# huyhoang17/DB_text_minimal

Measured on AMD Instinct MI355X. Metric: train images/sec @640x640 bs=16/GPU, higher is better.
Workload: dtype f32

## Files before the change

db_text_minimal_amd/_lib.py:

```python
import ctypes
import os
import subprocess

_HERE = os.path.dirname(os.path.abspath(__file__))
LIB_PATH = os.environ.get('DBN_LIB_PATH') or os.path.join(_HERE, 'libdbnet_hip.so')
CSRC = os.path.join(_HERE, 'csrc')

_P, _I, _L, _F = ctypes.c_void_p, ctypes.c_int, ctypes.c_long, ctypes.c_float

SIGNATURES = {
    'dbn_pack_weights': 'piiiiiipp',
    'dbn_igemm_panel_floats': 'iiiiii',
    'dbn_igemm_packed_floats': 'ii',
    'dbn_igemm_f32': 'pppp' + 'i' * 14 + 'p',
    'dbn_igemm_tile_config': 'ii',
    'dbn_igemm_tile_config_ns': 'iii',
    'dbn_conv_bn_ws_floats': 'iiiiii',
    'dbn_pack_weights_batched': 'piip',
    'dbn_igemm_splitk_plan': 'iiii',
    'dbn_igemm_splitk_plan_ns': 'iiiii',
    'dbn_igemm_splitk_f32': 'pppp' + 'i' * 16 + 'pp',
    'dbn_deform_im2col': 'ppp' + 'i' * 11 + 'p',
    'dbn_deform_col2im': 'ppppp' + 'i' + 'p' + 'i' * 11 + 'p',
    'dbn_deform_col2im_ws_bytes': 'i' * 8,
# ... 46 lines not shown
    'dbn_detect_poly': 'piiiifi' + 'pppppp',
    'dbn_detect_poly_host': 'ppppp' + 'iiii' + 'pp' + 'pppi' + 'pppp',
    'dbn_det_eval_ws_bytes': 'i',
    'dbn_det_eval_overlaps': 'ppipilippppp',
    'dbn_det_eval_match_host': 'ii' + 'p' * 12,
    'dbn_pyramid_conv_ws_floats': 'iiii',
    'dbn_pyramid_conv_f32': 'p' * 10 + 'i' * 7 + 'pp' + 'ff' + 'ppppppp' + 'p',
    'dbn_conv_bn_f32': 'pppp' + 'i' * 15 + 'pp' + 'ff' + 'ppppppp' + 'p',
    'dbn_pack_weights_bf16s': 'piiiiiiipp',
    'dbn_igemm_bf16s_panel_floats': 'iiiiiii',
    'dbn_igemm_bf16s': 'pppp' + 'i' * 15 + 'p',
    'dbn_wgrad_bf16s': 'pppp' + 'i' * 12 + 'fip',
    'dbn_wgrad_splitk': 'iiiiiii',
    'dbn_wgrad_slab_floats': 'iiiiiii',
    'dbn_wgrad_splitk_hw': 'iiiiiiiii',
    'dbn_wgrad_slab_floats_hw': 'iiiiiiiiii',
    'dbn_set_index_limits': 'lll',
    'dbn_wgrad_f32': 'pppp' + 'i' * 12 + 'fp',
    'dbn_reduce_ws_floats': 'i',
    'dbn_bn_train_stats': 'piippffppppppp' + 'p',
    'dbn_bn_eval_coef': 'ippppfppp',
    'dbn_bn_apply': 'pppppppliip',
    'dbn_bn_backward': 'pppppppp' + 'pp' + 'i' + 'pp' + 'ii' + 'f' + 'pp',
    'dbn_bn_backward_from_sums': 'ppppppppp' + 'pp' + 'i' + 'pp' + 'ii' + 'f' + 'pp',
    'dbn_bn_backward_ex': 'ppppppppp' + 'pp' + 'i' + 'ppp' + 'ii' + 'f' + 'pp',
    'dbn_col_sum': 'piipfpp',
    'dbn_bnrelu_maxpool_fwd': 'ppppiiiip',
    'dbn_bnrelu_maxpool_bwd': 'ppppppiiiip',
    'dbn_nearest_up_fwd': 'ppp' + 'i' * 8 + 'p',
    'dbn_nearest_up_bwd': 'pp' + 'i' * 9 + 'p',
    'dbn_bilinear_fwd': 'ppliiiip',
    'dbn_bilinear_bwd': 'ppliiiip',
    'dbn_fpn_combine_weights': 'piiiipp',
    'dbn_fpn_scatter_wgrad': 'ppppiipp',
    'dbn_nchw3_to_nhwc4': 'ppiiip',
    'dbn_add_inplace': 'pplp',
    'dbn_head_tail_fwd': 'p' * 11 + 'iiii' + 'f' + 'p',
    'dbn_head_tail_bwd_ws_floats': '',
    'dbn_head_tail_bwd': 'p' * 21 + 'iiii' + 'ff' + 'pp',
    'dbn_db_loss_ws_bytes': '',
    'dbn_db_loss_fwd': 'pp' + 'iiii' + 'ffff' + 'pppp',
    'dbn_db_loss_sum_fwd': 'pp' + 'iiii' + 'ffff' + 'pppp',
    'dbn_db_loss_frac_fwd': 'pp' + 'iiii' + 'ffff' + 'i' + 'pppp',
    'dbn_db_loss_bwd': 'pppp' + 'ff' + 'iiii' + 'pp',
    'dbn_db_loss_ohem_ws_bytes': 'iii',
    'dbn_db_loss_ohem_fwd': 'pp' + 'iiii' + 'ffff' + 'pppp',
    'dbn_db_loss_ohem_bwd': 'ppppp' + 'ff' + 'iiii' + 'pp',
    'dbn_pixel_confusion': 'plppiiifpp',
    'dbn_adam_step': 'pppp' + 'l' + 'ffff' + 'i' + 'f' + 'p',
    'dbn_clock_probe': 'pip',
    'dbn_has_experiments': '',
    'dbn_wall_clock_khz': '',
}
SIGNATURES.update({
    'dbn_igemm_t': 'ii' + 'pppp' + 'i' * 14 + 'i' + 'p' + 'p',
    'dbn_conv_bn_t': 'i' + SIGNATURES['dbn_conv_bn_f32'],
    'dbn_pyramid_conv_t': 'i' + SIGNATURES['dbn_pyramid_conv_f32'],
    'dbn_pyramid_conv_from_t': 'ii' + SIGNATURES['dbn_pyramid_conv_f32'],
    'dbn_igemm_bn_rows': 'i' * 15,
    'dbn_igemm_bnsums_t': 'ii' + 'pppp' + 'i' * 14 + 'ppppppp' + 'pppp' + 'p' + 'p',
    'dbn_igemm_bn_final_counters': 'ii',
    'dbn_igemm_bn_final_group_floats': 'ii',
    'dbn_wgrad_t': 'ii' + 'pppp' + 'i' * 12 + 'f' + 'p',
    'dbn_wgrad_phase_t': 'iii' + 'pppp' + 'i' * 12 + 'f' + 'p',
    'dbn_wgrad_reduce_describe': 'ii' + 'pppp' + 'i' * 12 + 'f' + 'p',
    'dbn_wgrad_reduce_many': 'ppiiip',
    'dbn_wgrad_tile_config': 'ii',
    'dbn_set_wgrad_variant': 'i',
    'dbn_set_convt_kernel': 'i',
    'dbn_igemm_splitk_slab_floats': 'iiiii',
    'dbn_wgrad_kernel_config': 'iiiii',
    'dbn_wgrad_kernel_config_hw': 'i' * 12,
    'dbn_set_patch_conv': 'i',
    'dbn_set_wres16': 'i',
    'dbn_set_pyramid_wide': 'i',
    'dbn_pyramid_wide_would_run': 'iiiiii',
    'dbn_conv_bn_set_final': 'pp',
    'dbn_conv_bn_final_group_doubles': 'ii',
    'dbn_wres16_would_run': 'iiiiiiiii',
    'dbn_mfma_sustained': 'ippip',
    'dbn_mfma_sustained_flops': 'ii',
    'dbn_set_stagger': 'i',
    'dbn_winograd_eligible': 'iiiii',
    'dbn_winograd_panel_floats': 'ii',
    'dbn_winograd_pack': 'piiiipp',
    'dbn_winograd_rows': 'iii',
    'dbn_winograd_pack_batched': 'pip',
    'dbn_winograd_dgrad_bnsums_f32': 'ppp' + 'iiiiii' + 'pppp' + 'ppp' + 'pppp' + 'p' + 'p',
    'dbn_winograd_ws_floats': 'iiii',
    'dbn_winograd_wgrad_eligible': 'iiiiii',
    'dbn_winograd_wgrad_linear': 'ii',
    'dbn_winograd_wgrad_slab_floats': 'iiiii',
    'dbn_winograd_wgrad_f32': 'ipppppp' + 'iiiiii' + 'fp',
    'dbn_winograd_conv_bn_act_f32': 'pppppp' + 'iiiii' + 'pp' + 'ff' + 'ppppppp' + 'p',
    'dbn_winograd_conv_bn_f32': 'pppp' + 'iiiii' + 'pp' + 'ff' + 'ppppppp' + 'p',
    'dbn_set_phase_priority': 'i',
    'dbn_set_winograd_persistent': 'i',
    'dbn_set_winograd_stagger': 'i',
    'dbn_set_winograd_blocks_per_barrier': 'i',
    'dbn_fold_bn_eval': 'pilppppp' + 'f' + 'ppp',
    'dbn_igemm_act_t': 'ii' + 'pppp' + 'i' + 'p' + 'i' * 13 + 'p',
    'dbn_winograd_conv_act_f32': 'pppp' + 'i' + 'p' + 'iiiii' + 'p',
    'dbn_pyramid_conv_act_t': 'ii' + 'p' * 9 + 'i' + 'p' + 'i' * 6 + 'p',
    'dbn_set_trace': 'pl',
    'dbn_igemm_kernel_config': 'i' * 16,
    'dbn_split3': 'pplp',
    'dbn_deform_im2col_t': 'i' + SIGNATURES['dbn_deform_im2col'],
    'dbn_deform_col2im_t': 'i' + SIGNATURES['dbn_deform_col2im'],
    'dbn_deform_col2im_gather_t': 'i' + SIGNATURES['dbn_deform_col2im'],
    'dbn_deform_col2im_gather_ws_bytes': 'iii',
    'dbn_deform_offset_absmax_t': 'iplpp',
    'dbn_pw16_eligible': 'iiiiii',
    'dbn_pw16_panel_bytes': '',
    'dbn_pw16_pack': 'ipipp',
    'dbn_pw16_act_t': 'ipppipiiiip',
    'dbn_set_head_tail_wide': 'i',
    'dbn_stem16_pool_eligible': 'iiii',
    'dbn_stem16_conv_bn_relu_pool_t': 'ipppppiiip',
    'dbn_head16_eligible': 'iiii',
    'dbn_head16_tail_eval_t': 'i' + 'p' * 15 + 'iii' + 'p',
    'dbn_cast_f32': 'ipplp',
    'dbn_pack_weights_t': 'ip' + 'i' * 7 + 'pp',
    'dbn_igemm_panel_floats_t': 'i' * 8,
    'dbn_bn_train_stats_t': 'i' + SIGNATURES['dbn_bn_train_stats'],
    'dbn_bn_apply_t': 'i' + SIGNATURES['dbn_bn_apply'],
    'dbn_bn_backward_t': 'ipi' + SIGNATURES['dbn_bn_backward_ex'][1:],
    'dbn_col_sum_t': 'i' + SIGNATURES['dbn_col_sum'],
    'dbn_bnrelu_maxpool_fwd_t': 'i' + SIGNATURES['dbn_bnrelu_maxpool_fwd'],
    'dbn_bnrelu_maxpool_bwd_t': 'i' + SIGNATURES['dbn_bnrelu_maxpool_bwd'][:-1] + 'pppp',
    'dbn_maxpool_bwd_parts': 'iiii',
    'dbn_bnrelu_maxpool_fwd_arg_t': 'ipppppp' + 'iiii' + 'p',
    'dbn_maxpool_bn_backward_ws_floats': 'iiii',
    'dbn_maxpool_bn_backward_t': 'i' + 'p' * 10 + 'iiii' + 'f' + 'pp',
    'dbn_nearest_up_fwd_t': 'i' + SIGNATURES['dbn_nearest_up_fwd'],
    'dbn_nearest_up_bwd_t': 'i' + SIGNATURES['dbn_nearest_up_bwd'],
    'dbn_nchw3_to_nhwc4_t': 'i' + SIGNATURES['dbn_nchw3_to_nhwc4'],
    'dbn_nchw3_to_nhwc4_packed_t': 'i' + SIGNATURES['dbn_nchw3_to_nhwc4'],
    'dbn_nchw3_to_nhwc16_and_4_t': 'ipppiiip',
    'dbn_convt16_rows': '',
    'dbn_convt16_panel_bytes': '',
    'dbn_convt16_eligible': 'iiiiii',
    'dbn_convt16_pack': 'ippp',
    'dbn_convt16_bn_t': 'ippppiii' + 'pp' + 'ff' + 'ppppppp' + 'p',
    'dbn_stem16_padded_h': 'i',
    'dbn_stem16_padded_w': 'i',
    'dbn_stem16_rows': '',
    'dbn_stem16_panel_bytes': '',
    'dbn_stem16_eligible': 'iiii',
    'dbn_stem16_pack': 'ippp',
    'dbn_nchw3_to_padded4_t': 'ipppiiip',
    'dbn_stem16_conv_bn_t': 'ipppiii' + 'pp' + 'ff' + 'ppppppp' + 'p',
    'dbn_head_tail_fwd_t': 'i' + SIGNATURES['dbn_head_tail_fwd'],
    'dbn_head_tail_bwd_t': 'i' + SIGNATURES['dbn_head_tail_bwd'],
})
LONG_RETURN = {'dbn_jpeg_coef_elems', 'dbn_jpeg_coef_elems_ex', 'dbn_jpeg_dhuff_ws_bytes', 'dbn_jpeg_encode_bound', 'dbn_greedy_decode_ws_bytes', 'dbn_det_eval_ws_bytes', 'dbn_detect_ws_bytes', 'dbn_detect_poly_ws_bytes', 'dbn_detect_poly_verts_cap', 'dbn_mfma_sustained_flops', 'dbn_conv_bn_final_group_doubles', 'dbn_maxpool_bn_backward_ws_floats', 'dbn_pw16_panel_bytes', 'dbn_stem16_panel_bytes', 'dbn_convt16_panel_bytes', 'dbn_winograd_panel_floats', 'dbn_winograd_wgrad_slab_floats', 'dbn_winograd_ws_floats', 'dbn_igemm_splitk_slab_floats', 'dbn_deform_col2im_ws_bytes', 'dbn_deform_col2im_gather_ws_bytes', 'dbn_igemm_bn_final_counters', 'dbn_igemm_bn_final_group_floats', 'dbn_igemm_panel_floats_t', 'dbn_wgrad_slab_floats_hw', 'dbn_wgrad_slab_floats', 'dbn_igemm_panel_floats', 'dbn_igemm_bf16s_panel_floats', 'dbn_db_loss_ohem_ws_bytes', 'dbn_conv_bn_ws_floats', 'dbn_pyramid_conv_ws_floats'}
_KIND = {'p': _P, 'i': _I, 'l': _L, 'f': _F}


class HipLibraryError(RuntimeError):
    pass


class WgradReduceJob(ctypes.Structure):
    _fields_ = ([('slab', _P), ('grad', _P)] + [(f, _I) for f in ('splitk', 'O', 'J', 'Jp', 'BM', 'BN', 'Cb', 'I', 'RS', 'G', 'natural', 'blocks')]
                + [('scale', _F), ('smem_bytes', _I)])


class BnbFinal(ctypes.Structure):
    _fields_ = [('counters', _P), ('group', _P), ('c1c2', _P), ('dgamma', _P), ('dbeta', _P), ('c1c2_2', _P), ('dgamma_2', _P),
                ('dbeta_2', _P), ('grad_scale', _F)]


def build(verbose=False):
    res = subprocess.run(['make', '-C', CSRC, '-j8'], capture_output=True, text=True)
    if verbose or res.returncode != 0:
        print(res.stdout[-4000:])
        print(res.stderr[-4000:])
    if res.returncode != 0:
        raise HipLibraryError('building libdbnet_hip.so failed (see output above)')
    return LIB_PATH


def source_stamp():
    import hashlib
    h = hashlib.sha256()
    for name in sorted(os.listdir(CSRC)):
        if name.endswith(('.hip', '.h')) or name == 'Makefile':
            h.update(name.encode())
            with open(os.path.join(CSRC, name), 'rb') as f:
                h.update(f.read())
    return h.hexdigest()[:16]


_lib = None


def lib():
    global _lib
    if _lib is None:
        if not os.path.exists(LIB_PATH):
            raise HipLibraryError('%s not found: run `python -c "import __graft_entry__ as g; g.build()"` '
                                  '(there is no CPU fallback for the DBNet hot path)' % LIB_PATH)
        try:
            l = ctypes.CDLL(LIB_PATH)
        except OSError as e:
            raise HipLibraryError('cannot load %s: %s' % (LIB_PATH, e))
        for name, sig in SIGNATURES.items():
            fn = getattr(l, name)
            fn.argtypes = [_KIND[k] for k in sig]
            fn.restype = _L if name in LONG_RETURN else _I
        _lib = l
    return _lib


def check(rc, what=''):
    if rc != 0:
        if rc == 1:
            raise RuntimeError('libdbnet_hip: invalid argument in %s' % what)
        raise RuntimeError('libdbnet_hip: %s failed with hipError %d' % (what, rc - 1000))
```

db_text_minimal_amd/csrc/head_loss.hip:

```cpp
#include "common.h"

namespace {

__device__ __forceinline__ float sigmoidf_(float x) { return 1.f / (1.f + __expf(-x)); }
__device__ __forceinline__ float sigmoid_acc(float x) { return 1.f / (1.f + expf(-x)); }
__device__ __forceinline__ float sigmoid_fast(float x) { return __builtin_amdgcn_rcpf(1.f + __expf(-x)); }

template <int CTRL>
__device__ __forceinline__ float dpp_f32(float v) {
    return __builtin_bit_cast(float, __builtin_amdgcn_update_dpp(0, __builtin_bit_cast(int, v), CTRL, 0xF, 0xF, true));
}
constexpr int DPP_QUAD_XOR1 = 0xB1;
constexpr int DPP_QUAD_XOR2 = 0x4E;
constexpr int DPP_ROW_HALF_MIRROR = 0x141;
constexpr int DPP_ROW_MIRROR = 0x140;
__device__ __forceinline__ float group16_sum(float v) {
    v += dpp_f32<DPP_QUAD_XOR1>(v);
    v += dpp_f32<DPP_QUAD_XOR2>(v);
    v += dpp_f32<DPP_ROW_HALF_MIRROR>(v);
    v += dpp_f32<DPP_ROW_MIRROR>(v);
    return v;
}
#ifndef DBN_HT_NODPP
#define DBN_HT_NODPP 0
#endif
#ifndef DBN_HT_CHECK
#define DBN_HT_CHECK 0
#endif
#ifndef DBN_HT_WAVES
#define DBN_HT_WAVES 0
#endif
template <int K>
__device__ __forceinline__ float quad_bcast(float v) {
#if DBN_HT_NODPP
    return __shfl(v, (int)((threadIdx.x & 63u & ~3u) | K), 64);
#else
    return dpp_f32<K | (K << 2) | (K << 4) | (K << 6)>(v);
#endif
}

__device__ __forceinline__ float group8_sum(float v) {
    v += dpp_f32<DPP_QUAD_XOR1>(v);
    v += dpp_f32<DPP_QUAD_XOR2>(v);
    v += dpp_f32<DPP_ROW_HALF_MIRROR>(v);
    return v;
}

template <int AT, int LPP>
__global__ __launch_bounds__(256) void head_tail_fwd_kernel(const void* __restrict__ xb, const void* __restrict__ xt, const float* __restrict__ wb,
                                     const float* __restrict__ wt, const float* __restrict__ bias_b,
                                     const float* __restrict__ bias_t, const float* __restrict__ sc_b,
                                     const float* __restrict__ sh_b, const float* __restrict__ sc_t,
                                     const float* __restrict__ sh_t, float* __restrict__ out, int N, int Hq, int Wq, int CH,
                                     float kstep, long per) {
    static_assert((LPP == 16) || (LPP == 8 && AT != 0), "eight lanes per pixel: 16-bit storage");
    constexpr int NQ = 16 / LPP;
    const int q = threadIdx.x & (LPP - 1);
    const bool bn = sc_b != nullptr;
    f32x4 scb[NQ], shb[NQ], sct[NQ], sht[NQ];
#pragma unroll
    for (int h = 0; h < NQ; ++h) {
        scb[h] = sct[h] = f32x4{1.f, 1.f, 1.f, 1.f};
        shb[h] = sht[h] = f32x4{0.f, 0.f, 0.f, 0.f};
        if (bn) {
            scb[h] = *reinterpret_cast<const f32x4*>(sc_b + 4 * (NQ * q + h));
            shb[h] = *reinterpret_cast<const f32x4*>(sh_b + 4 * (NQ * q + h));
            sct[h] = *reinterpret_cast<const f32x4*>(sc_t + 4 * (NQ * q + h));
            sht[h] = *reinterpret_cast<const f32x4*>(sh_t + 4 * (NQ * q + h));
        }
    }
    const long npx = (long)N * Hq * Wq;
    const long gstride = blockDim.x / LPP;
    const long r1 = min(npx, (blockIdx.x + 1) * per);
    f32x4 wbq[4 * NQ], wtq[4 * NQ];
#pragma unroll
    for (int e = 0; e < 4 * NQ; ++e) {
        wbq[e] = *reinterpret_cast<const f32x4*>(wb + (4 * NQ * q + e) * 4);
        wtq[e] = *reinterpret_cast<const f32x4*>(wt + (4 * NQ * q + e) * 4);
    }
    const float bb = bias_b[0], bt = bias_t[0];
    const int H = 2 * Hq, W = 2 * Wq;
    const long HW = (long)H * W;
    const long px0 = blockIdx.x * per + (threadIdx.x / LPP);
    const long HWq = (long)Hq * Wq;
    long n = px0 / HWq;
    int hq = (int)((px0 - n * HWq) / Wq), wq = (int)((px0 - n * HWq) - (long)hq * Wq);
    const long g_n = gstride / HWq;
    const int g_h = (int)((gstride - g_n * HWq) / Wq), g_w = (int)((gstride - g_n * HWq) - (long)g_h * Wq);
    auto advance = [&]() {
        wq += g_w;
        if (wq >= Wq) { wq -= Wq; ++hq; }
        hq += g_h;
        if (hq >= Hq) { hq -= Hq; ++n; }
        n += g_n;
    };
    auto load = [&](const void* x, long px, f32x4 (&v)[NQ]) {
        if constexpr (NQ == 1) v[0] = dbn_ld4<AT>(x, px * 16 + q);
        else dbn_ldq<AT>(x, px * 8 + q, v);
    };
    auto finish = [&](f32x4 (&vb)[NQ], f32x4 (&vt)[NQ], long pn, int ph, int pw) {
        if (bn) {
#pragma unroll
            for (int h = 0; h < NQ; ++h)
#pragma unroll
                for (int e = 0; e < 4; ++e) {
                    vb[h][e] = dbn_affine_relu(vb[h][e], scb[h][e], shb[h][e]);
                    vt[h][e] = dbn_affine_relu(vt[h][e], sct[h][e], sht[h][e]);
                }
        }
        f32x4 sb = {0.f, 0.f, 0.f, 0.f}, stt = {0.f, 0.f, 0.f, 0.f};
#pragma unroll
        for (int h = 0; h < NQ; ++h)
#pragma unroll
            for (int e = 0; e < 4; ++e) {
                sb += vb[h][e] * wbq[4 * h + e];
                stt += vt[h][e] * wtq[4 * h + e];
            }
#pragma unroll
        for (int ab = 0; ab < 4; ++ab) {
            sb[ab] = LPP == 16 ? group16_sum(sb[ab]) : group8_sum(sb[ab]);
            stt[ab] = LPP == 16 ? group16_sum(stt[ab]) : group8_sum(stt[ab]);
        }
        if (q < 4) {
            const int ab = q;
            const float lp = (ab == 0 ? sb[0] : ab == 1 ? sb[1] : ab == 2 ? sb[2] : sb[3]) + bb;
            const float lt = (ab == 0 ? stt[0] : ab == 1 ? stt[1] : ab == 2 ? stt[2] : stt[3]) + bt;
            const float P = sigmoid_fast(lp), T = sigmoid_fast(lt);
            const long o = (long)(2 * ph + (ab >> 1)) * W + 2 * pw + (ab & 1);
            float* base = out + pn * CH * HW + o;
            base[0] = P;
            base[HW] = T;
            if (CH == 3) base[2 * HW] = sigmoid_fast(kstep * (P - T));
        }
    };
    long px = px0;
    for (; px + 3 * gstride < r1; px += 4 * gstride) {
        f32x4 vb[4][NQ], vt[4][NQ];
#pragma unroll
        for (int u = 0; u < 4; ++u) {
            load(xb, px + u * gstride, vb[u]);
            load(xt, px + u * gstride, vt[u]);
        }
#pragma unroll
        for (int u = 0; u < 4; ++u) {
            finish(vb[u], vt[u], n, hq, wq);
            advance();
        }
    }
    for (; px < r1; px += gstride, advance()) {
        f32x4 vb[NQ], vt[NQ];
        load(xb, px, vb);
        load(xt, px, vt);
        finish(vb, vt, n, hq, wq);
    }
}

#if DBN_HT_WAVES
#define DBN_HT_OCC __attribute__((amdgpu_waves_per_eu(DBN_HT_WAVES, DBN_HT_WAVES)))
#else
#define DBN_HT_OCC
#endif
template <int AT>
__global__ __launch_bounds__(256) DBN_HT_OCC void head_tail_bwd_kernel(const void* __restrict__ xb, const void* __restrict__ xt, const float* __restrict__ wb,
                                     const float* __restrict__ wt, const float* __restrict__ preds,
                                     const float* __restrict__ dpreds, const float* __restrict__ sc_b,
                                     const float* __restrict__ sh_b, const float* __restrict__ sc_t,
                                     const float* __restrict__ sh_t, const float* __restrict__ mean_b,
                                     const float* __restrict__ rstd_b, const float* __restrict__ mean_t,
                                     const float* __restrict__ rstd_t, void* __restrict__ dxb, void* __restrict__ dxt,
                                     float* __restrict__ part, int N, int Hq, int Wq, int CH, float kstep) {
    const int q = threadIdx.x & 15;
    const int grp = threadIdx.x >> 4;
    const bool bn = sc_b != nullptr;
    f32x4 scb = {1.f, 1.f, 1.f, 1.f}, shb = {0.f, 0.f, 0.f, 0.f}, sct = scb, sht = shb;
    if (bn) {
        scb = *reinterpret_cast<const f32x4*>(sc_b + 4 * q);
        shb = *reinterpret_cast<const f32x4*>(sh_b + 4 * q);
        sct = *reinterpret_cast<const f32x4*>(sc_t + 4 * q);
        sht = *reinterpret_cast<const f32x4*>(sh_t + 4 * q);
    }
    const long npx = (long)N * Hq * Wq;
    const long gstride = (long)gridDim.x * (blockDim.x >> 4);
    f32x4 wbq[4], wtq[4];
#pragma unroll
    for (int e = 0; e < 4; ++e) {
        wbq[e] = *reinterpret_cast<const f32x4*>(wb + (4 * q + e) * 4);
        wtq[e] = *reinterpret_cast<const f32x4*>(wt + (4 * q + e) * 4);
    }
    const bool bnsum = bn && mean_b != nullptr;
    f32x4 mub = {0.f, 0.f, 0.f, 0.f}, rsb = mub, mut = mub, rst = mub;
    if (bnsum) {
        mub = *reinterpret_cast<const f32x4*>(mean_b + 4 * q);
        rsb = *reinterpret_cast<const f32x4*>(rstd_b + 4 * q);
        mut = *reinterpret_cast<const f32x4*>(mean_t + 4 * q);
        rst = *reinterpret_cast<const f32x4*>(rstd_t + 4 * q);
    }
    f32x4 s1b = {0.f, 0.f, 0.f, 0.f}, s2b = s1b, s1t = s1b, s2t = s1b;
    const int H = 2 * Hq, W = 2 * Wq;
    const long HW = (long)H * W;
    f32x4 awb[4], awt[4];
#pragma unroll
    for (int e = 0; e < 4; ++e) {
        awb[e] = f32x4{0.f, 0.f, 0.f, 0.f};
        awt[e] = f32x4{0.f, 0.f, 0.f, 0.f};
    }
    float abb = 0.f, abt = 0.f;
    const long px0 = blockIdx.x * (long)(blockDim.x >> 4) + grp;
    const long HWq = (long)Hq * Wq;
    long n = px0 / HWq;
    int hq = (int)((px0 - n * HWq) / Wq), wq = (int)((px0 - n * HWq) - (long)hq * Wq);
    const long g_n = gstride / HWq;
    const int g_h = (int)((gstride - g_n * HWq) / Wq), g_w = (int)((gstride - g_n * HWq) - (long)g_h * Wq);
    auto advance = [&]() {
        wq += g_w;
        if (wq >= Wq) { wq -= Wq; ++hq; }
        hq += g_h;
        if (hq >= Hq) { hq -= Hq; ++n; }
        n += g_n;
    };
    for (long px = px0; px < npx; px += gstride, advance()) {
        float dlb = 0.f, dlt = 0.f;
        {
            const int ab = q & 3;
            const long o = (long)(2 * hq + (ab >> 1)) * W + 2 * wq + (ab & 1);
            const float* pb = preds + n * CH * HW + o;
            const float* db = dpreds + n * CH * HW + o;
            const float P = pb[0], T = pb[HW];
            float dP = db[0], dT = db[HW];
            if (CH == 3) {
                const float B = pb[2 * HW];
                const float gB = db[2 * HW] * kstep * B * (1.f - B);
                dP += gB;
                dT -= gB;
            }
            dlb = dP * P * (1.f - P);
            dlt = dT * T * (1.f - T);
        }
        const f32x4 lb = {quad_bcast<0>(dlb), quad_bcast<1>(dlb), quad_bcast<2>(dlb), quad_bcast<3>(dlb)};
        const f32x4 lt = {quad_bcast<0>(dlt), quad_bcast<1>(dlt), quad_bcast<2>(dlt), quad_bcast<3>(dlt)};
        f32x4 vb = dbn_ld4<AT>(xb, px * 16 + q);
        f32x4 vt = dbn_ld4<AT>(xt, px * 16 + q);
        const f32x4 yb = vb, yt = vt;
        if (bn) {
#pragma unroll
            for (int e = 0; e < 4; ++e) {
                vb[e] = dbn_affine_relu(vb[e], scb[e], shb[e]);
                vt[e] = dbn_affine_relu(vt[e], sct[e], sht[e]);
            }
        }
        f32x4 gb, gt;
#pragma unroll
        for (int e = 0; e < 4; ++e) {
            gb[e] = wbq[e][0] * lb[0] + wbq[e][1] * lb[1] + wbq[e][2] * lb[2] + wbq[e][3] * lb[3];
            gt[e] = wtq[e][0] * lt[0] + wtq[e][1] * lt[1] + wtq[e][2] * lt[2] + wtq[e][3] * lt[3];
            awb[e] += vb[e] * lb;
            awt[e] += vt[e] * lt;
        }
        dbn_st4<AT>(dxb, px * 16 + q, gb);
        dbn_st4<AT>(dxt, px * 16 + q, gt);
        if (bnsum) {
            if constexpr (AT != 0) {
#pragma unroll
                for (int e = 0; e < 4; ++e) {
                    gb[e] = AT == 1 ? (float)(__bf16)gb[e] : (float)(_Float16)gb[e];
                    gt[e] = AT == 1 ? (float)(__bf16)gt[e] : (float)(_Float16)gt[e];
                }
            }
#pragma unroll
            for (int e = 0; e < 4; ++e) {
                const float mb = vb[e] > 0.f ? gb[e] : 0.f, mt = vt[e] > 0.f ? gt[e] : 0.f;
                s1b[e] += mb;
                s2b[e] += mb * ((yb[e] - mub[e]) * rsb[e]);
                s1t[e] += mt;
                s2t[e] += mt * ((yt[e] - mut[e]) * rst[e]);
            }
        }
        if (q == 0) {
            abb += lb[0] + lb[1] + lb[2] + lb[3];
            abt += lt[0] + lt[1] + lt[2] + lt[3];
        }
    }
#if DBN_HT_CHECK
    {
        float* dbg = part + (long)(2 * 257 + 4 * 64) * gridDim.x;
        int bad_w = 0, bad_t = 0, low_only = 0;
#pragma unroll
        for (int e = 0; e < 4; ++e) {
            const f32x4 a = *reinterpret_cast<const volatile f32x4*>(wb + (4 * q + e) * 4), b = *reinterpret_cast<const volatile f32x4*>(wt + (4 * q + e) * 4);
#pragma unroll
            for (int k = 0; k < 4; ++k) {
                const unsigned ua = __builtin_bit_cast(unsigned, a[k]), ur = __builtin_bit_cast(unsigned, wbq[e][k]);
                bad_w += ua != ur;
                low_only += (ua != ur) && ((ua >> 16) == (ur >> 16));
                bad_t += __builtin_bit_cast(unsigned, b[k]) != __builtin_bit_cast(unsigned, wtq[e][k]);
            }
        }
        int bad_s = 0;
        if (bn) {
            const f32x4 a = *reinterpret_cast<const volatile f32x4*>(sc_b + 4 * q), b = *reinterpret_cast<const volatile f32x4*>(sh_b + 4 * q);
#pragma unroll
            for (int k = 0; k < 4; ++k) bad_s += (__builtin_bit_cast(unsigned, a[k]) != __builtin_bit_cast(unsigned, scb[k])) + (__builtin_bit_cast(unsigned, b[k]) != __builtin_bit_cast(unsigned, shb[k]));
        }
        if (bad_w) atomicAdd(dbg + 0, 1.f);
        if (bad_t) atomicAdd(dbg + 1, 1.f);
        if (bad_s) atomicAdd(dbg + 2, 1.f);
        if (low_only) atomicAdd(dbg + 4, 1.f);
    }
#endif
    constexpr int ROWS = 2 * 257 + 4 * 64;
    __shared__ float red[16][ROWS];
    {
        float* r = red[grp];
#pragma unroll
        for (int e = 0; e < 4; ++e)
#pragma unroll
            for (int ab = 0; ab < 4; ++ab) {
                r[(4 * q + e) * 4 + ab] = awb[e][ab];
                r[257 + (4 * q + e) * 4 + ab] = awt[e][ab];
            }
        if (q == 0) {
            r[256] = abb;
            r[257 + 256] = abt;
        }
#pragma unroll
        for (int e = 0; e < 4; ++e) {
            r[514 + 4 * q + e] = s1b[e];
            r[514 + 64 + 4 * q + e] = s2b[e];
            r[514 + 128 + 4 * q + e] = s1t[e];
            r[514 + 192 + 4 * q + e] = s2t[e];
        }
    }
    __syncthreads();
    for (int i = threadIdx.x; i < ROWS; i += blockDim.x) {
        float s = 0.f;
        for (int g = 0; g < 16; ++g) s += red[g][i];
        part[(long)i * gridDim.x + blockIdx.x] = s;
    }
}

__global__ void fold_partials_d_kernel(const float* __restrict__ part, int nb, int n, float* __restrict__ out, float scale) {
    const int i = blockIdx.x * 8 + (threadIdx.x >> 5);
    const int l32 = threadIdx.x & 31;
    if (i >= n) return;
    const double s = dbn_team32_fold(part, nb, i, l32);
    if (l32 == 0) out[i] = (float)(s * scale);
}

__global__ void fold_head_grads_kernel(const float* __restrict__ part, int nb, float* __restrict__ dw_b, float* __restrict__ dbias_b,
                                       float* __restrict__ dw_t, float* __restrict__ dbias_t, float scale) {
    const int i = blockIdx.x * 8 + (threadIdx.x >> 5);
    const int l32 = threadIdx.x & 31;
    if (i >= 2 * 257) return;
    const double s = dbn_team32_fold(part, nb, i, l32);
    if (l32 != 0) return;
    const int j = i < 257 ? i : i - 257;
    float* dst = i < 257 ? (j < 256 ? dw_b + j : dbias_b) : (j < 256 ? dw_t + j : dbias_t);
    *dst = (float)(s * scale);
}

enum { S_POS = 0, S_NEG, S_BCE, S_L1, S_A, S_BGM, S_BM, S_NONBIN , NSUM };

template <int V>
__device__ __forceinline__ f32x4 ldv(const float* p) {
    if constexpr (V == 4) return *reinterpret_cast<const f32x4*>(p);
    return f32x4{p[0], 0.f, 0.f, 0.f};
}
template <int V>
__device__ __forceinline__ void stv(float* p, f32x4 v) {
    if constexpr (V == 4) *reinterpret_cast<f32x4*>(p) = v;
    else p[0] = v[0];
}



struct DbLossFinal {
    long px;
    int CH;
    float alpha, beta, negative_ratio, eps;
    int bce_sum;
    float* losses;
    float* coef;
    unsigned* counter;
};

__device__ __forceinline__ void db_loss_finish(const double (&s)[NSUM], const DbLossFinal& f) {
    const long n_pos = (long)(float)s[S_POS];
    const long n_neg_expect = (long)((double)n_pos * (double)f.negative_ratio);
    const long n_neg_cur = (long)(float)s[S_NEG];
    const long n_neg = n_neg_expect < n_neg_cur ? n_neg_expect : n_neg_cur;
    const double bce_div = f.bce_sum ? 1.0 : (double)f.px;
    const float bce = (float)(s[S_BCE] / bce_div);
    const float denom = (float)((double)(n_pos + n_neg) + (double)f.eps);
    const float num_w = (float)s[S_POS] + (float)n_neg;
    const float prob = bce * num_w / denom;
    const float thr = (float)s[S_L1] / ((float)s[S_A] + f.eps);
    const float pt = prob + f.beta * thr;
    float* losses = f.losses;
    float* coef = f.coef;
    losses[0] = prob;
    losses[1] = thr;
    coef[0] = num_w / denom / (float)bce_div;
    coef[1] = 1.f / ((float)s[S_A] + f.eps);
    coef[7] = (float)s[S_NONBIN];
    if (f.CH == 3) {
        const float U = (float)s[S_BM] + (float)s[S_POS] + f.eps;
        const float I = (float)s[S_BGM];
        const float binl = 1.f - 2.f * I / U;
        losses[2] = binl;
        losses[3] = pt;
        losses[4] = f.alpha * binl + pt;
        coef[2] = U;
        coef[3] = I;
    } else {
        losses[2] = 0.f;
        losses[3] = pt;
        losses[4] = pt;
        coef[2] = 1.f;
        coef[3] = 0.f;
    }
}

__device__ __forceinline__ void db_loss_fold_and_finish(const double* __restrict__ part, int nb, const DbLossFinal& f, double* red ) {
    constexpr int PER = 4;
    double v[PER][NSUM];
#pragma unroll
    for (int i = 0; i < PER; ++i) {
        const int b = threadIdx.x + i * 256;
#pragma unroll
        for (int k = 0; k < NSUM; ++k)
            v[i][k] = (b < nb && threadIdx.x < 256) ? __hip_atomic_load(part + (long)b * NSUM + k, __ATOMIC_RELAXED, __HIP_MEMORY_SCOPE_AGENT) : 0.0;
    }
    const int lane = threadIdx.x & 63, wave = threadIdx.x >> 6;
    __syncthreads();
#pragma unroll
    for (int k = 0; k < NSUM; ++k) {
        const double w = dbn_wave_sum_d((v[0][k] + v[1][k]) + (v[2][k] + v[3][k]));
        if (lane == 0 && wave < 4) red[wave * 8 + k] = w;
    }
    __syncthreads();
    if (threadIdx.x != 0) return;
    double s[NSUM];
    for (int k = 0; k < NSUM; ++k) s[k] = (red[k] + red[8 + k]) + (red[16 + k] + red[24 + k]);
    db_loss_finish(s, f);
}

__device__ __forceinline__ float bce_term(float x, float t) {
    if (t == 1.f || t == 0.f) {
        const bool pos = t == 1.f;
        const float u = -x, w = pos ? x : 1.f + u;
        float l = __logf(w);
        if (!pos) l = (w == 1.f) ? u : l * (u * __builtin_amdgcn_rcpf(w - 1.f));
        return -fmaxf(l, -100.f);
    }
    const float lp = fmaxf(logf(x), -100.f);
    const float lq = fmaxf(log1pf(-x), -100.f);
    return (t - 1.f) * lq - t * lp;
}

template <int V>
__global__ void db_loss_fwd_kernel(const float* __restrict__ preds, const float* __restrict__ gts, int N, long HW, int CH,
                                   double* __restrict__ part, DbLossFinal fin) {
    const long total4 = (long)N * HW / V;
    const long NHW = (long)N * HW;
    float s[NSUM];
#pragma unroll
    for (int k = 0; k < NSUM; ++k) s[k] = 0.f;
    double ds[NSUM];
#pragma unroll
    for (int k = 0; k < NSUM; ++k) ds[k] = 0.0;
    int cnt = 0;
    for (long i = blockIdx.x * (long)blockDim.x + threadIdx.x; i < total4; i += (long)gridDim.x * blockDim.x) {
        const long p = i * V;
        const long n = p / HW, o = p - n * HW;
        const float* pb = preds + n * CH * HW + o;
        const f32x4 P = ldv<V>(pb);
        const f32x4 T = ldv<V>(pb + HW);
        f32x4 B = {0.f, 0.f, 0.f, 0.f};
        if (CH == 3) B = ldv<V>(pb + 2 * HW);
        const f32x4 G = ldv<V>(gts + p);
        const f32x4 M = ldv<V>(gts + NHW + p);
        const f32x4 Tg = ldv<V>(gts + 2 * NHW + p);
        const f32x4 A = ldv<V>(gts + 3 * NHW + p);
#pragma unroll
        for (int e = 0; e < V; ++e) {
            s[S_POS] += G[e] * M[e];
            s[S_NEG] += (1.f - G[e]) * M[e];
            s[S_BCE] += bce_term(P[e], G[e]);
            s[S_L1] += fabsf(T[e] - Tg[e]) * A[e];
            s[S_A] += A[e];
            s[S_BGM] += B[e] * G[e] * M[e];
            s[S_BM] += B[e] * M[e];
            s[S_NONBIN] += (G[e] * (1.f - G[e]) != 0.f || M[e] * (1.f - M[e]) != 0.f) ? 1.f : 0.f;
        }
        if (++cnt == 64) {
#pragma unroll
            for (int k = 0; k < NSUM; ++k) {
                ds[k] += (double)s[k];
                s[k] = 0.f;
            }
            cnt = 0;
        }
    }
#pragma unroll
    for (int k = 0; k < NSUM; ++k) ds[k] += (double)s[k];
    __shared__ double red[8][8];
    __shared__ int s_last;
    const int lane = threadIdx.x & 63, wave = threadIdx.x >> 6;
#pragma unroll
    for (int k = 0; k < NSUM; ++k) {
        const double w = dbn_wave_sum_d(ds[k]);
// ... 200 lines not shown
                                     int frac, double bce_div) {
    if (threadIdx.x != 0 || blockIdx.x != 0) return;
    double s_pos = 0.0, pos_loss = 0.0, sel = 0.0, cnt_gt = 0.0, s_bce = 0.0;
    for (int b = 0; b < nb_sums; ++b) s_pos += part_sums[(long)b * NSUM + S_POS];
    if (frac)
        for (int b = 0; b < nb_sums; ++b) s_bce += part_sums[(long)b * NSUM + S_BCE];
    for (int b = 0; b < nb_pos; ++b) pos_loss += part_pos[b];
    for (int b = 0; b < nb_sel; ++b) {
        sel += part_sel[2 * b];
        cnt_gt += part_sel[2 * b + 1];
    }
    const double k = (double)st[0];
    const float tau = k > 0 ? __builtin_bit_cast(float, (unsigned)st[3]) : 0.f;
    const double n_tie = k - cnt_gt;
    const double cnt_eq = (double)st[4];
    const long n_pos = (long)(float)s_pos;
    const float denom = (float)((double)n_pos + k + (double)eps);
    float prob = (float)(pos_loss + sel + n_tie * (double)tau) / denom;
    if (frac) {
        const float bce = (float)(s_bce / bce_div);
        const float num_w = (float)(pos_loss + sel + n_tie * (double)tau);
        prob = bce * num_w / denom;
        const float thr_f = losses[1], pt_f = prob + beta * thr_f;
        losses[0] = prob;
        losses[3] = pt_f;
        losses[4] = (CH == 3 ? alpha * losses[2] : 0.f) + pt_f;
        coef[0] = num_w / denom / (float)bce_div;
        coef[7] = 0.f;
        return;
    }
    const float thr = losses[1];
    const float pt = prob + beta * thr;
    losses[0] = prob;
    losses[3] = pt;
    losses[4] = (CH == 3 ? alpha * losses[2] : 0.f) + pt;
    coef[0] = 1.f / denom;
    coef[4] = k > 0 ? tau : 3.0e38f;
    coef[5] = (k > 0 && cnt_eq > 0) ? (float)(n_tie / cnt_eq) : 0.f;
    coef[6] = 1.f;
}

__global__ void pixel_confusion_kernel(const float* __restrict__ preds, long batch_stride, const float* __restrict__ gt,
                                       const float* __restrict__ mask, int N, long HW, float thresh, double* __restrict__ hist) {
    const long total = (long)N * HW;
    unsigned c01 = 0, c10 = 0, c11 = 0;
    for (long i = blockIdx.x * (long)blockDim.x + threadIdx.x; i < total; i += (long)gridDim.x * blockDim.x) {
        const long n = i / HW, o = i - n * HW;
        const float m = mask[i];
        const int p = preds[n * batch_stride + o] * m > thresh;
        const int g = (int)(gt[i] * m) != 0;
        c01 += (!g) & p;
        c10 += g & (!p);
        c11 += g & p;
    }
    __shared__ unsigned red[4][3];
    const int lane = threadIdx.x & 63, wave = threadIdx.x >> 6;
    unsigned v[3] = {c01, c10, c11};
#pragma unroll
    for (int k = 0; k < 3; ++k) {
#pragma unroll
        for (int o = 32; o > 0; o >>= 1) v[k] += __shfl_xor(v[k], o, 64);
        if (lane == 0) red[wave][k] = v[k];
    }
    __syncthreads();
    if (threadIdx.x < 3) {
        unsigned t = 0;
        for (int w = 0; w < (int)(blockDim.x >> 6); ++w) t += red[w][threadIdx.x];
        atomicAdd(&hist[1 + threadIdx.x], (double)t);
    }
    if (blockIdx.x == 0 && threadIdx.x == 3) atomicAdd(&hist[4], (double)total);
}

}

extern "C" {

static int g_head_tail_wide = 0;
int dbn_set_head_tail_wide(int mode) {
    const int old = g_head_tail_wide;
    g_head_tail_wide = mode > 0 ? 1 : mode < 0 ? -1 : 0;
    return old;
}
int dbn_head_tail_fwd_t(int at, const void* xb, const void* xt, const float* wb, const float* wt, const float* bias_b,
                        const float* bias_t, const float* bn_scale_b, const float* bn_shift_b, const float* bn_scale_t,
                        const float* bn_shift_t, float* out, int N, int Hq, int Wq, int channels, float kstep, void* stream) {
    DBN_REQUIRE(xb && xt && wb && wt && bias_b && bias_t && out && (channels == 2 || channels == 3));
    DBN_REQUIRE((bn_scale_b && bn_shift_b && bn_scale_t && bn_shift_t) || (!bn_scale_b && !bn_shift_b && !bn_scale_t && !bn_shift_t));
    const long npx = (long)N * Hq * Wq;
    const long per = ((npx + 16383) / 16384 + 63) / 64 * 64;
    const dim3 grid((unsigned)((npx + per - 1) / per));
    const bool wide = (at == 1 || at == 2) && (g_head_tail_wide > 0 || (g_head_tail_wide == 0 && npx >= (1L << 22)));
    if (wide && at == 1)
        hipLaunchKernelGGL((head_tail_fwd_kernel<1, 8>), grid, dim3(256), 0, (hipStream_t)stream, xb, xt, wb, wt, bias_b, bias_t, bn_scale_b,
                           bn_shift_b, bn_scale_t, bn_shift_t, out, N, Hq, Wq, channels, kstep, per);
    else if (wide && at == 2)
        hipLaunchKernelGGL((head_tail_fwd_kernel<2, 8>), grid, dim3(256), 0, (hipStream_t)stream, xb, xt, wb, wt, bias_b, bias_t, bn_scale_b,
                           bn_shift_b, bn_scale_t, bn_shift_t, out, N, Hq, Wq, channels, kstep, per);
    else if (at == 1)
        hipLaunchKernelGGL((head_tail_fwd_kernel<1, 16>), grid, dim3(256), 0, (hipStream_t)stream, xb, xt, wb, wt, bias_b, bias_t, bn_scale_b,
                           bn_shift_b, bn_scale_t, bn_shift_t, out, N, Hq, Wq, channels, kstep, per);
    else if (at == 2)
        hipLaunchKernelGGL((head_tail_fwd_kernel<2, 16>), grid, dim3(256), 0, (hipStream_t)stream, xb, xt, wb, wt, bias_b, bias_t, bn_scale_b,
                           bn_shift_b, bn_scale_t, bn_shift_t, out, N, Hq, Wq, channels, kstep, per);
    else if (at == 0)
        hipLaunchKernelGGL((head_tail_fwd_kernel<0, 16>), grid, dim3(256), 0, (hipStream_t)stream, xb, xt, wb, wt, bias_b, bias_t, bn_scale_b,
                           bn_shift_b, bn_scale_t, bn_shift_t, out, N, Hq, Wq, channels, kstep, per);
    else
        return DBN_ERR_ARG;
    return dbn_status();
}
int dbn_head_tail_fwd(const float* xb, const float* xt, const float* wb, const float* wt, const float* bias_b,
                      const float* bias_t, const float* bn_scale_b, const float* bn_shift_b, const float* bn_scale_t,
                      const float* bn_shift_t, float* out, int N, int Hq, int Wq, int channels, float kstep, void* stream) {
    return dbn_head_tail_fwd_t(0, xb, xt, wb, wt, bias_b, bias_t, bn_scale_b, bn_shift_b, bn_scale_t, bn_shift_t, out, N, Hq, Wq,
                               channels, kstep, stream);
}

int dbn_head_tail_bwd_ws_floats() { return 2048 * (2 * 257 + 4 * 64); }

int dbn_head_tail_bwd_t(int at, const void* xb, const void* xt, const float* wb, const float* wt, const float* preds,
                        const float* dpreds, const float* bn_scale_b, const float* bn_shift_b, const float* bn_scale_t,
                        const float* bn_shift_t, const float* bn_mean_b, const float* bn_rstd_b, const float* bn_mean_t,
                        const float* bn_rstd_t, float* bn_sums, void* dxb, void* dxt, float* dw_b, float* dbias_b, float* dw_t,
                        float* dbias_t, int N, int Hq, int Wq, int channels, float kstep, float grad_scale, float* ws, void* stream) {
    DBN_REQUIRE(xb && xt && wb && wt && preds && dpreds && dxb && dxt && dw_b && dbias_b && dw_t && dbias_t && ws);
    DBN_REQUIRE((bn_scale_b && bn_shift_b && bn_scale_t && bn_shift_t) || (!bn_scale_b && !bn_shift_b && !bn_scale_t && !bn_shift_t));
    DBN_REQUIRE(channels == 2 || channels == 3);
    const bool sums = bn_sums != nullptr;
    DBN_REQUIRE(!sums || (bn_scale_b && bn_mean_b && bn_rstd_b && bn_mean_t && bn_rstd_t));
    hipStream_t st = (hipStream_t)stream;
    const long npx = (long)N * Hq * Wq;
    const int nb = dbn_grid(npx * 16, 256, 2047);
    DBN_DISPATCH_AT(at, hipLaunchKernelGGL(head_tail_bwd_kernel<AT>, dim3(nb), dim3(256), 0, st, xb, xt, wb, wt, preds, dpreds, bn_scale_b,
                                           bn_shift_b, bn_scale_t, bn_shift_t, sums ? bn_mean_b : nullptr, bn_rstd_b, bn_mean_t,
                                           bn_rstd_t, dxb, dxt, ws, N, Hq, Wq, channels, kstep));
    hipLaunchKernelGGL(fold_head_grads_kernel, dim3(dbn_ceil_div(2 * 257, 8)), dim3(256), 0, st, ws, nb, dw_b, dbias_b, dw_t, dbias_t,
                       grad_scale);
    if (sums)
        hipLaunchKernelGGL(fold_partials_d_kernel, dim3(dbn_ceil_div(256, 8)), dim3(256), 0, st, ws + (long)514 * nb, nb, 256, bn_sums,
                           1.0f);
    return dbn_status();
}

int dbn_head_tail_bwd(const float* xb, const float* xt, const float* wb, const float* wt, const float* preds,
                      const float* dpreds, const float* bn_scale_b, const float* bn_shift_b, const float* bn_scale_t,
                      const float* bn_shift_t, const float* bn_mean_b, const float* bn_rstd_b, const float* bn_mean_t,
                      const float* bn_rstd_t, float* bn_sums, float* dxb, float* dxt, float* dw_b, float* dbias_b, float* dw_t,
                      float* dbias_t, int N, int Hq, int Wq, int channels, float kstep, float grad_scale, float* ws, void* stream) {
    return dbn_head_tail_bwd_t(0, xb, xt, wb, wt, preds, dpreds, bn_scale_b, bn_shift_b, bn_scale_t, bn_shift_t, bn_mean_b, bn_rstd_b,
                               bn_mean_t, bn_rstd_t, bn_sums, dxb, dxt, dw_b, dbias_b, dw_t, dbias_t, N, Hq, Wq, channels, kstep,
                               grad_scale, ws, stream);
}

static const long DB_LOSS_PART_BYTES = 1024L * NSUM * 8;
int dbn_db_loss_ws_bytes() { return (int)DB_LOSS_PART_BYTES + 64; }

static const long OHEM_OFF_POS = DB_LOSS_PART_BYTES + 64, OHEM_OFF_SEL = OHEM_OFF_POS + 1024L * 8, OHEM_OFF_ST = OHEM_OFF_SEL + 2048L * 8,
                  OHEM_OFF_HIST = OHEM_OFF_ST + 64, OHEM_OFF_V = OHEM_OFF_HIST + 3L * OHEM_BINS * 4;
long dbn_db_loss_ohem_ws_bytes(int N, int H, int W) { return OHEM_OFF_V + (long)N * H * W * 4; }

static int db_loss_fwd_run(const float* preds, const float* gts, int N, int H, int W, int channels, float alpha, float beta,
                           float negative_ratio, float eps, int per_pixel, float* losses, float* coef, void* ws, void* stream) {
    DBN_REQUIRE(preds && gts && losses && coef && ws && (channels == 2 || channels == 3));
    const long HW = (long)H * W;
    hipStream_t st = (hipStream_t)stream;
    const bool vec = HW % 4 == 0;
    const int nb = dbn_grid((long)N * HW / (vec ? 4 : 1), 512, 1024);
    char* base = (char*)ws;
    const int frac = per_pixel >= 3, bce_sum = (per_pixel == 2 || per_pixel == 4) ? 1 : 0;
    DbLossFinal fin = {(long)N * HW, channels, alpha, beta, negative_ratio, eps, bce_sum, losses, coef,
                       (unsigned*)(base + DB_LOSS_PART_BYTES)};
    if (hipMemsetAsync(fin.counter, 0, sizeof(unsigned), st) != hipSuccess) return dbn_status();
    if (vec)
        hipLaunchKernelGGL(db_loss_fwd_kernel<4>, dim3(nb), dim3(512), 0, st, preds, gts, N, HW, channels, (double*)ws, fin);
    else
        hipLaunchKernelGGL(db_loss_fwd_kernel<1>, dim3(nb), dim3(512), 0, st, preds, gts, N, HW, channels, (double*)ws, fin);
    if (per_pixel != 1 && !frac) return dbn_status();
    double* part_pos = (double*)(base + OHEM_OFF_POS);
    double* part_sel = (double*)(base + OHEM_OFF_SEL);
    unsigned long long* state = (unsigned long long*)(base + OHEM_OFF_ST);
    unsigned* hist = (unsigned*)(base + OHEM_OFF_HIST);
    float* v = (float*)(base + OHEM_OFF_V);
    const long total = (long)N * HW;
    const int nbv = dbn_grid(total, 256, 1024);
    hipLaunchKernelGGL(ohem_prepare_kernel, dim3(1), dim3(256), 0, st, (const double*)ws, nb, negative_ratio, state, hist);
    hipLaunchKernelGGL(ohem_values_kernel, dim3(nbv), dim3(256), 0, st, preds, gts, N, HW, channels, v, part_pos, frac);
    for (int pass = 0; pass < 3; ++pass) {
        hipLaunchKernelGGL(ohem_hist_kernel, dim3(nbv), dim3(256), 0, st, v, total, state, pass, hist);
        hipLaunchKernelGGL(ohem_scan_kernel, dim3(1), dim3(64), 0, st, state, hist, pass);
    }
    hipLaunchKernelGGL(ohem_sum_kernel, dim3(nbv), dim3(256), 0, st, v, total, state, part_sel);
    hipLaunchKernelGGL(ohem_finalize_kernel, dim3(1), dim3(64), 0, st, (const double*)ws, nb, part_pos, nbv, part_sel, nbv, state,
                       channels, alpha, beta, eps, losses, coef, frac, bce_sum ? 1.0 : (double)((long)N * HW));
    return dbn_status();
}

int dbn_db_loss_fwd(const float* preds, const float* gts, int N, int H, int W, int channels, float alpha, float beta,
                    float negative_ratio, float eps, float* losses, float* coef, void* ws, void* stream) {
    return db_loss_fwd_run(preds, gts, N, H, W, channels, alpha, beta, negative_ratio, eps, 0, losses, coef, ws, stream);
}

int dbn_db_loss_sum_fwd(const float* preds, const float* gts, int N, int H, int W, int channels, float alpha, float beta,
                        float negative_ratio, float eps, float* losses, float* coef, void* ws, void* stream) {
    return db_loss_fwd_run(preds, gts, N, H, W, channels, alpha, beta, negative_ratio, eps, 2, losses, coef, ws, stream);
}

int dbn_db_loss_ohem_fwd(const float* preds, const float* gts, int N, int H, int W, int channels, float alpha, float beta,
                         float negative_ratio, float eps, float* losses, float* coef, void* ws, void* stream) {
    return db_loss_fwd_run(preds, gts, N, H, W, channels, alpha, beta, negative_ratio, eps, 1, losses, coef, ws, stream);
}

int dbn_db_loss_frac_fwd(const float* preds, const float* gts, int N, int H, int W, int channels, float alpha, float beta,
                         float negative_ratio, float eps, int sum, float* losses, float* coef, void* ws, void* stream) {
    return db_loss_fwd_run(preds, gts, N, H, W, channels, alpha, beta, negative_ratio, eps, sum ? 4 : 3, losses, coef, ws, stream);
}

static int db_loss_bwd_run(const float* preds, const float* gts, const float* coef, const float* grad_losses, const float* ohem_v,
                           float alpha, float beta, int N, int H, int W, int channels, float* dpreds, void* stream) {
    DBN_REQUIRE(preds && gts && coef && grad_losses && dpreds && (channels == 2 || channels == 3));
    const long HW = (long)H * W;
    if (HW % 4 == 0)
        hipLaunchKernelGGL(db_loss_bwd_kernel<4>, dim3(dbn_grid((long)N * HW / 4)), dim3(256), 0, (hipStream_t)stream, preds, gts,
                           coef, grad_losses, ohem_v, alpha, beta, N, HW, channels, dpreds);
    else
        hipLaunchKernelGGL(db_loss_bwd_kernel<1>, dim3(dbn_grid((long)N * HW)), dim3(256), 0, (hipStream_t)stream, preds, gts, coef,
                           grad_losses, ohem_v, alpha, beta, N, HW, channels, dpreds);
    return dbn_status();
}

int dbn_db_loss_bwd(const float* preds, const float* gts, const float* coef, const float* grad_losses, float alpha, float beta,
                    int N, int H, int W, int channels, float* dpreds, void* stream) {
    return db_loss_bwd_run(preds, gts, coef, grad_losses, nullptr, alpha, beta, N, H, W, channels, dpreds, stream);
}

int dbn_db_loss_ohem_bwd(const float* preds, const float* gts, const float* coef, const float* grad_losses, const void* ws,
                         float alpha, float beta, int N, int H, int W, int channels, float* dpreds, void* stream) {
    DBN_REQUIRE(ws);
    return db_loss_bwd_run(preds, gts, coef, grad_losses, (const float*)((const char*)ws + OHEM_OFF_V), alpha, beta, N, H, W, channels,
                           dpreds, stream);
}

int dbn_pixel_confusion(const float* preds, long batch_stride, const float* gt, const float* mask, int N, int H, int W, float thresh,
                        double* hist, void* stream) {
    DBN_REQUIRE(preds && gt && mask && hist && N > 0 && H > 0 && W > 0);
    const long total = (long)N * H * W;
    hipLaunchKernelGGL(pixel_confusion_kernel, dim3(dbn_grid(total, 256, 2048)), dim3(256), 0, (hipStream_t)stream, preds, batch_stride,
                       gt, mask, N, (long)H * W, thresh, hist);
    return dbn_status();
}

}
```

db_text_minimal_amd/csrc/pointwise.hip:

```cpp
#include "common.h"

namespace {

constexpr int MAX_PART = 1024;
constexpr int STREAM_BLOCKS = 768;
constexpr int UNROLL = 4;

constexpr int CHUNK_C = 1024;

template <int NV, class F>
__device__ __forceinline__ void channel_reduce(int M, int Cfull, float* __restrict__ part, F&& body) {
    const int cb = blockIdx.y * CHUNK_C, C = min(CHUNK_C, Cfull - cb);
    const int c4n = C >> 2, cq = cb >> 2;
    const int c4 = threadIdx.x % c4n, rl = threadIdx.x / c4n;
    const int nrl = blockDim.x / c4n;
    const int rows_per = (M + gridDim.x - 1) / gridDim.x;
    const int r0 = blockIdx.x * rows_per, r1 = min(M, r0 + rows_per);
    f32x4 acc[NV];
#pragma unroll
    for (int v = 0; v < NV; ++v) acc[v] = f32x4{0.f, 0.f, 0.f, 0.f};
    if (rl < nrl) {
#pragma unroll 4
        for (int r = r0 + rl; r < r1; r += nrl) body(r, cq + c4, acc);
    }
    extern __shared__ float red[];
    if (rl < nrl) {
#pragma unroll
        for (int v = 0; v < NV; ++v) *reinterpret_cast<f32x4*>(red + ((long)rl * NV + v) * C + 4 * c4) = acc[v];
    }
    __syncthreads();
    for (int i = threadIdx.x; i < NV * C; i += blockDim.x) {
        float s = 0.f;
        for (int k = 0; k < nrl; ++k) s += red[(long)k * NV * C + i];
        const int v = i / C, c = i - v * C;
        part[((long)v * Cfull + cb + c) * gridDim.x + blockIdx.x] = s;
    }
}

template <int AT>
__global__ void bn_stats_kernel(const void* __restrict__ y, int M, int C, float* __restrict__ part) {
    const int c4n = C >> 2;
    channel_reduce<2>(M, C, part, [&](int r, int c4, f32x4* acc) {
        const f32x4 pv = dbn_ld4<AT>(y, c4);
        const f32x4 v = dbn_ld4<AT>(y, (long)r * c4n + c4) - pv;
        acc[0] += v;
        acc[1] += v * v;
    });
}

template <int AT>
__global__ void bn_finalize_kernel(const float* __restrict__ part, int nb, const void* __restrict__ y, int M, int C,
                                   const float* __restrict__ gamma, const float* __restrict__ beta, float eps, float momentum,
                                   float* __restrict__ run_mean, float* __restrict__ run_var, float* __restrict__ scale,
                                   float* __restrict__ shift, float* __restrict__ mean_out, float* __restrict__ rstd_out) {
    const int c = blockIdx.x * 8 + (threadIdx.x >> 5);
    const int l32 = threadIdx.x & 31;
    if (c >= C) return;
    const double s1 = dbn_team32_fold(part, nb, c, l32);
    const double s2 = dbn_team32_fold(part, nb, (long)C + c, l32);
    if (l32 != 0) return;
    const double pv = (double)dbn_ld1<AT>(y, c);
    const double dm = s1 / M;
    const double mean = pv + dm;
    double var = s2 / M - dm * dm;
    if (var < 0.0) var = 0.0;
    const float rstd = (float)(1.0 / sqrt(var + (double)eps));
    const float meanf = (float)mean;
    const float sc = gamma[c] * rstd;
    scale[c] = sc;
    shift[c] = fmaf(-meanf, sc, beta[c]);
    mean_out[c] = meanf;
    rstd_out[c] = rstd;
    if (run_mean) {
        const double unb = M > 1 ? var * ((double)M / (double)(M - 1)) : var;
        run_mean[c] = (1.f - momentum) * run_mean[c] + momentum * meanf;
        run_var[c] = (1.f - momentum) * run_var[c] + momentum * (float)unb;
    }
}

__global__ void bn_eval_coef_kernel(int C, const float* __restrict__ gamma, const float* __restrict__ beta,
                                    const float* __restrict__ run_mean, const float* __restrict__ run_var, float eps,
                                    float* __restrict__ scale, float* __restrict__ shift) {
    const int c = blockIdx.x * blockDim.x + threadIdx.x;
    if (c >= C) return;
    const float rstd = 1.f / sqrtf(run_var[c] + eps);
    const float sc = gamma[c] * rstd;
    scale[c] = sc;
    shift[c] = fmaf(-run_mean[c], sc, beta[c]);
}

template <int AT, int QW>
__global__ __launch_bounds__(256) void bn_apply_kernel(const void* __restrict__ y, const float* __restrict__ sc,
                                                       const float* __restrict__ sh, const void* __restrict__ res,
                                                       const float* __restrict__ rsc, const float* __restrict__ rsh,
                                                       void* __restrict__ out, long total, int C, int relu) {
    static_assert(QW == 1 || (QW == 2 && AT != 0), "two quads per access: 16-bit storage");
    const int cin = C / (4 * QW);
    const long i0 = blockIdx.x * (long)blockDim.x + threadIdx.x;
    const long stride = (long)gridDim.x * blockDim.x;
    const int c = (int)(i0 % cin) * 4 * QW;
    f32x4 s[QW], h[QW], s2[QW], h2[QW];
#pragma unroll
    for (int q = 0; q < QW; ++q) {
        s[q] = *reinterpret_cast<const f32x4*>(sc + c + 4 * q);
        h[q] = *reinterpret_cast<const f32x4*>(sh + c + 4 * q);
        s2[q] = s[q];
        h2[q] = h[q];
        if (res && rsc) {
            s2[q] = *reinterpret_cast<const f32x4*>(rsc + c + 4 * q);
            h2[q] = *reinterpret_cast<const f32x4*>(rsh + c + 4 * q);
        }
    }
    auto ld = [&](const void* ptr, long i, f32x4 (&v)[QW]) {
        if constexpr (QW == 1) v[0] = dbn_ld4<AT>(ptr, i);
        else dbn_ldq<AT>(ptr, i, v);
    };
    auto st = [&](long i, const f32x4 (&v)[QW]) {
        if constexpr (QW == 1) dbn_st4<AT>(out, i, v[0]);
        else dbn_stq<AT>(out, i, v);
    };
    auto one = [&](long i, const f32x4 (&v)[QW], const f32x4 (&r)[QW]) {
        f32x4 o[QW];
#pragma unroll
        for (int q = 0; q < QW; ++q) {
#pragma unroll
            for (int e = 0; e < 4; ++e) o[q][e] = dbn_affine(v[q][e], s[q][e], h[q][e]);
            if (res) {
                if (rsc) {
#pragma unroll
                    for (int e = 0; e < 4; ++e) o[q][e] += dbn_affine(r[q][e], s2[q][e], h2[q][e]);
                } else {
                    o[q] += r[q];
                }
            }
            if (relu) {
#pragma unroll
                for (int e = 0; e < 4; ++e) o[q][e] = fmaxf(o[q][e], 0.f);
            }
        }
        st(i, o);
    };
    const f32x4 zero = {0.f, 0.f, 0.f, 0.f};
    long i = i0;
    for (; i + (UNROLL - 1) * stride < total; i += UNROLL * stride) {
        f32x4 v[UNROLL][QW], r[UNROLL][QW];
#pragma unroll
        for (int u = 0; u < UNROLL; ++u) ld(y, i + u * stride, v[u]);
#pragma unroll
        for (int u = 0; u < UNROLL; ++u) {
            if (res) ld(res, i + u * stride, r[u]);
            else {
#pragma unroll
                for (int q = 0; q < QW; ++q) r[u][q] = zero;
            }
        }
#pragma unroll
        for (int u = 0; u < UNROLL; ++u) one(i + u * stride, v[u], r[u]);
    }
    for (; i < total; i += stride) {
        f32x4 v[QW], r[QW];
        ld(y, i, v);
        if (res) ld(res, i, r);
        else {
#pragma unroll
            for (int q = 0; q < QW; ++q) r[q] = zero;
        }
        one(i, v, r);
    }
}

template <int AT>
__global__ void bn_bwd_reduce_kernel(const void* __restrict__ y, const void* __restrict__ zmask, const float* __restrict__ msc,
                                     const float* __restrict__ msh, const void* __restrict__ dout,
                                     const float* __restrict__ mean, const float* __restrict__ rstd, int M, int C,
                                     float* __restrict__ part) {
    const int c4n = C >> 2;
    channel_reduce<2>(M, C, part, [&](int r, int c4, f32x4* acc) {
        const long off = (long)r * c4n + c4;
        f32x4 g = dbn_ld4<AT>(dout, off);
        const f32x4 v = dbn_ld4<AT>(y, off);
        if (zmask) {
            const f32x4 z = dbn_ld4<AT>(zmask, off);
#pragma unroll
            for (int e = 0; e < 4; ++e) g[e] = z[e] > 0.f ? g[e] : 0.f;
        } else if (msc) {
            const f32x4 s_ = *reinterpret_cast<const f32x4*>(msc + 4 * c4);
            const f32x4 h_ = *reinterpret_cast<const f32x4*>(msh + 4 * c4);
#pragma unroll
            for (int e = 0; e < 4; ++e) g[e] = dbn_affine(v[e], s_[e], h_[e]) > 0.f ? g[e] : 0.f;
        }
        const f32x4 mu = *reinterpret_cast<const f32x4*>(mean + 4 * c4);
        const f32x4 rs = *reinterpret_cast<const f32x4*>(rstd + 4 * c4);
        acc[0] += g;
        acc[1] += g * ((v - mu) * rs);
    });
}

__global__ void bn_bwd_finalize_kernel(const float* __restrict__ part, int nb, int M, int C, float* __restrict__ dgamma,
                                       float* __restrict__ dbeta, float* __restrict__ c1, float* __restrict__ c2, float gscale) {
    const int c = blockIdx.x * 8 + (threadIdx.x >> 5);
    const int l32 = threadIdx.x & 31;
    if (c >= C) return;
    const double s1 = dbn_team32_fold(part, nb, c, l32);
    const double s2 = dbn_team32_fold(part, nb, (long)C + c, l32);
    if (l32 != 0) return;
    dbeta[c] = (float)(s1 * gscale);
    dgamma[c] = (float)(s2 * gscale);
    c1[c] = (float)(s1 / M);
    c2[c] = (float)(s2 / M);
}

__global__ __launch_bounds__(256) void bn_bwd_finalize_wide_kernel(const float* __restrict__ part, int nb, int M, int C,
                                                                   float* __restrict__ dgamma, float* __restrict__ dbeta,
                                                                   float* __restrict__ c1, float* __restrict__ c2, float gscale) {
    __shared__ double red[2][256];
    const int c = blockIdx.x, t = threadIdx.x;
    const float* p1 = part + (long)c * nb;
    const float* p2 = part + ((long)C + c) * nb;
    double s1 = 0.0, s2 = 0.0;
    int b = t;
    for (; b + 768 < nb; b += 1024) {
        const float a0 = p1[b], a1 = p1[b + 256], a2 = p1[b + 512], a3 = p1[b + 768];
        const float q0 = p2[b], q1 = p2[b + 256], q2 = p2[b + 512], q3 = p2[b + 768];
        s1 += ((double)a0 + (double)a1) + ((double)a2 + (double)a3);
        s2 += ((double)q0 + (double)q1) + ((double)q2 + (double)q3);
    }
    for (; b < nb; b += 256) {
        s1 += (double)p1[b];
        s2 += (double)p2[b];
    }
    red[0][t] = s1;
    red[1][t] = s2;
    __syncthreads();
    for (int o = 128; o > 0; o >>= 1) {
        if (t < o) {
            red[0][t] += red[0][t + o];
            red[1][t] += red[1][t + o];
        }
        __syncthreads();
    }
    if (t != 0) return;
    s1 = red[0][0];
    s2 = red[1][0];
    dbeta[c] = (float)(s1 * gscale);
    dgamma[c] = (float)(s2 * gscale);
    c1[c] = (float)(s1 / M);
    c2[c] = (float)(s2 / M);
}

template <int AT>
__device__ __forceinline__ float round_to_storage(float v) {
    if constexpr (AT == 1) return (float)(__bf16)v;
    else if constexpr (AT == 2) return (float)(_Float16)v;
    else return v;
}

template <int AT, int QW>
__global__ __launch_bounds__(256) void bn_bwd_apply_kernel(const void* __restrict__ y, const void* __restrict__ zmask,
                                                           const float* __restrict__ msc, const float* __restrict__ msh,
                                                           const void* __restrict__ dout, const float* __restrict__ mean,
                                                           const float* __restrict__ rstd, const float* __restrict__ gamma,
                                                           const float* __restrict__ c1, const float* __restrict__ c2,
                                                           void* __restrict__ dy, void* __restrict__ gout, int gout_acc,
                                                           long total, int C, float* __restrict__ bias_part) {
    static_assert(QW == 1 || (QW == 2 && AT != 0), "two quads per access: 16-bit storage");
    const int cin = C / (4 * QW);
    const long i0 = blockIdx.x * (long)blockDim.x + threadIdx.x;
    const long stride = (long)gridDim.x * blockDim.x;
    const int c = (int)(i0 % cin) * 4 * QW;
    const f32x4 zero = {0.f, 0.f, 0.f, 0.f};
    f32x4 s_[QW], h_[QW], mu[QW], rs[QW], k1[QW], k2[QW], gr[QW], bsum[QW];
#pragma unroll
    for (int q = 0; q < QW; ++q) {
        s_[q] = h_[q] = zero;
        if (msc) {
            s_[q] = *reinterpret_cast<const f32x4*>(msc + c + 4 * q);
            h_[q] = *reinterpret_cast<const f32x4*>(msh + c + 4 * q);
        }
        mu[q] = *reinterpret_cast<const f32x4*>(mean + c + 4 * q);
        rs[q] = *reinterpret_cast<const f32x4*>(rstd + c + 4 * q);
        k1[q] = *reinterpret_cast<const f32x4*>(c1 + c + 4 * q);
        k2[q] = *reinterpret_cast<const f32x4*>(c2 + c + 4 * q);
        gr[q] = *reinterpret_cast<const f32x4*>(gamma + c + 4 * q) * rs[q];
        bsum[q] = zero;
    }
    const bool acc = gout && gout_acc;
    auto ld = [&](const void* ptr, long i, f32x4 (&v)[QW]) {
        if constexpr (QW == 1) v[0] = dbn_ld4<AT>(ptr, i);
        else dbn_ldq<AT>(ptr, i, v);
    };
    auto st = [&](void* ptr, long i, const f32x4 (&v)[QW]) {
        if constexpr (QW == 1) dbn_st4<AT>(ptr, i, v[0]);
        else dbn_stq<AT>(ptr, i, v);
    };
    auto one = [&](long i, f32x4 (&g)[QW], const f32x4 (&v)[QW], const f32x4 (&z)[QW], const f32x4 (&old)[QW]) {
        f32x4 d[QW], go[QW];
#pragma unroll
        for (int q = 0; q < QW; ++q) {
            if (zmask) {
#pragma unroll
                for (int e = 0; e < 4; ++e) g[q][e] = z[q][e] > 0.f ? g[q][e] : 0.f;
            } else if (msc) {
#pragma unroll
                for (int e = 0; e < 4; ++e) g[q][e] = dbn_affine(v[q][e], s_[q][e], h_[q][e]) > 0.f ? g[q][e] : 0.f;
            }
            const f32x4 xh = (v[q] - mu[q]) * rs[q];
            d[q] = gr[q] * (g[q] - k1[q] - xh * k2[q]);
#pragma unroll
            for (int e = 0; e < 4; ++e) {
                float t = d[q][e];
                asm("" : "+v"(t));
                d[q][e] = round_to_storage<AT>(t);
            }
            bsum[q] += d[q];
            go[q] = acc ? g[q] + old[q] : g[q];
        }
        st(dy, i, d);
        if (gout) st(gout, i, go);
    };
    auto zeros = [&](f32x4 (&v)[QW]) {
#pragma unroll
        for (int q = 0; q < QW; ++q) v[q] = zero;
    };
    long i = i0;
    for (; i + (UNROLL - 1) * stride < total; i += UNROLL * stride) {
        f32x4 g[UNROLL][QW], v[UNROLL][QW], z[UNROLL][QW], o[UNROLL][QW];
#pragma unroll
        for (int u = 0; u < UNROLL; ++u) {
            ld(dout, i + u * stride, g[u]);
            ld(y, i + u * stride, v[u]);
        }
#pragma unroll
        for (int u = 0; u < UNROLL; ++u) {
            if (zmask) ld(zmask, i + u * stride, z[u]);
            else zeros(z[u]);
            if (acc) ld(gout, i + u * stride, o[u]);
            else zeros(o[u]);
        }
#pragma unroll
        for (int u = 0; u < UNROLL; ++u) one(i + u * stride, g[u], v[u], z[u], o[u]);
    }
    for (; i < total; i += stride) {
        f32x4 g[QW], v[QW], z[QW], o[QW];
        ld(dout, i, g);
        ld(y, i, v);
        if (zmask) ld(zmask, i, z);
        else zeros(z);
        if (acc) ld(gout, i, o);
        else zeros(o);
        one(i, g, v, z, o);
    }
    if (bias_part) {
        __shared__ f32x4 red[QW][256];
#pragma unroll
        for (int q = 0; q < QW; ++q) red[q][threadIdx.x] = bsum[q];
        __syncthreads();
        if ((int)threadIdx.x < cin) {
            const int cq = (int)((blockIdx.x * (long)blockDim.x + threadIdx.x) % cin) * 4 * QW;
#pragma unroll
            for (int q = 0; q < QW; ++q) {
                f32x4 t = zero;
                for (int k = threadIdx.x; k < 256; k += cin) t += red[q][k];
#pragma unroll
                for (int e = 0; e < 4; ++e) bias_part[(long)(cq + 4 * q + e) * gridDim.x + blockIdx.x] = t[e];
            }
        }
    }
}

template <int AT>
__global__ void col_sum_kernel(const void* __restrict__ x, int M, int C, float* __restrict__ part) {
    const int c4n = C >> 2;
    channel_reduce<1>(M, C, part, [&](int r, int c4, f32x4* acc) { acc[0] += dbn_ld4<AT>(x, (long)r * c4n + c4); });
}

__global__ void fold_partials_kernel(const float* __restrict__ part, int nb, int n, float* __restrict__ out, float scale) {
    const int i = blockIdx.x * 8 + (threadIdx.x >> 5);
    const int l32 = threadIdx.x & 31;
    if (i >= n) return;
    const double s = dbn_team32_fold(part, nb, i, l32);
    if (l32 == 0) out[i] = (float)(s * scale);
}

template <int AT, int QW>
__global__ void bnrelu_maxpool_fwd_kernel(const void* __restrict__ y, const float* __restrict__ sc, const float* __restrict__ sh,
                                          void* __restrict__ out, int N, int H, int W, int C, int Ho, int Wo) {
    static_assert(QW == 1 || (QW == 2 && AT != 0), "two quads per access: 16-bit storage");
    const int cin = C / (4 * QW);
    const int Hp = (Ho + 1) >> 1;
    const long total = (long)N * Hp * Wo * cin;
    auto ld = [&](long i, f32x4 (&v)[QW]) {
        if constexpr (QW == 1) v[0] = dbn_ld4<AT>(y, i);
        else dbn_ldq<AT>(y, i, v);
    };
    auto st = [&](long i, const f32x4 (&v)[QW]) {
        if constexpr (QW == 1) dbn_st4<AT>(out, i, v[0]);
        else dbn_stq<AT>(out, i, v);
    };
    for (long i = blockIdx.x * (long)blockDim.x + threadIdx.x; i < total; i += (long)gridDim.x * blockDim.x) {
        const int ci = (int)(i % cin);
        long t = i / cin;
        const int ow = (int)(t % Wo);
        t /= Wo;
        const int k = (int)(t % Hp);
        const int n = (int)(t / Hp);
        f32x4 s[QW], h[QW], m0[QW], m1[QW];
#pragma unroll
        for (int q = 0; q < QW; ++q) {
            s[q] = *reinterpret_cast<const f32x4*>(sc + 4 * (QW * ci + q));
            h[q] = *reinterpret_cast<const f32x4*>(sh + 4 * (QW * ci + q));
            m0[q] = m1[q] = f32x4{0.f, 0.f, 0.f, 0.f};
        }
#pragma unroll
        for (int r = 0; r < 5; ++r) {
            const int ih = 4 * k - 1 + r;
            if ((unsigned)ih >= (unsigned)H) continue;
            f32x4 rm[QW];
#pragma unroll
            for (int q = 0; q < QW; ++q) rm[q] = f32x4{0.f, 0.f, 0.f, 0.f};
#pragma unroll
            for (int qq = 0; qq < 3; ++qq) {
                const int iw = ow * 2 - 1 + qq;
                if ((unsigned)iw >= (unsigned)W) continue;
                f32x4 v[QW];
                ld((((long)n * H + ih) * W + iw) * cin + ci, v);
#pragma unroll
                for (int q = 0; q < QW; ++q)
#pragma unroll
                    for (int e = 0; e < 4; ++e) rm[q][e] = fmaxf(rm[q][e], dbn_affine_relu(v[q][e], s[q][e], h[q][e]));
            }
#pragma unroll
            for (int q = 0; q < QW; ++q)
#pragma unroll
                for (int e = 0; e < 4; ++e) {
                    if (r <= 2) m0[q][e] = fmaxf(m0[q][e], rm[q][e]);
                    if (r >= 2) m1[q][e] = fmaxf(m1[q][e], rm[q][e]);
                }
        }
        const long o = (((long)n * Ho + 2 * k) * Wo + ow) * cin + ci;
        st(o, m0);
        if (2 * k + 1 < Ho) st(o + (long)Wo * cin, m1);
    }
}

template <int AT, int QW>
__global__ void bnrelu_maxpool_bwd_kernel(const void* __restrict__ y, const float* __restrict__ sc, const float* __restrict__ sh,
                                          const void* __restrict__ pooled, const void* __restrict__ dpool,
                                          void* __restrict__ dz, int N, int H, int W, int C, int Ho, int Wo,
                                          const float* __restrict__ mean, const float* __restrict__ rstd, float* __restrict__ bn_part) {
    static_assert(QW == 1 || (QW == 2 && AT != 0), "two quads per access: 16-bit storage");
    const int cin = C / (4 * QW);
    const int Hb = (H + 1) >> 1, Wb = (W + 1) >> 1;
    const long total = (long)N * Hb * Wb * cin;
    const f32x4 zero = {0.f, 0.f, 0.f, 0.f};
    f32x4 s1[QW], s2[QW], mu[QW], rs[QW];
    const int cq0 = (int)((blockIdx.x * (long)blockDim.x + threadIdx.x) % cin) * 4 * QW;
#pragma unroll
    for (int q = 0; q < QW; ++q) {
        s1[q] = s2[q] = mu[q] = rs[q] = zero;
        if (bn_part) {
            mu[q] = *reinterpret_cast<const f32x4*>(mean + cq0 + 4 * q);
            rs[q] = *reinterpret_cast<const f32x4*>(rstd + cq0 + 4 * q);
        }
    }
    auto ld = [&](const void* ptr, long i, f32x4 (&v)[QW]) {
        if constexpr (QW == 1) v[0] = dbn_ld4<AT>(ptr, i);
        else dbn_ldq<AT>(ptr, i, v);
    };
    for (long i = blockIdx.x * (long)blockDim.x + threadIdx.x; i < total; i += (long)gridDim.x * blockDim.x) {
        const int ci = (int)(i % cin);
        long t = i / cin;
        const int b = (int)(t % Wb);
        t /= Wb;
        const int a = (int)(t % Hb);
        const int n = (int)(t / Hb);
        f32x4 s[QW], h[QW];
#pragma unroll
        for (int q = 0; q < QW; ++q) {
            s[q] = *reinterpret_cast<const f32x4*>(sc + 4 * (QW * ci + q));
            h[q] = *reinterpret_cast<const f32x4*>(sh + 4 * (QW * ci + q));
        }
        f32x4 pm[2][2][QW], dp[2][2][QW];
        bool wok[2][2];
#pragma unroll
        for (int u = 0; u < 2; ++u)
#pragma unroll
            for (int w = 0; w < 2; ++w) {
                wok[u][w] = a + u < Ho && b + w < Wo;
                const long o = (((long)n * Ho + a + u) * Wo + b + w) * cin + ci;
#pragma unroll
                for (int q = 0; q < QW; ++q) pm[u][w][q] = dp[u][w][q] = zero;
                if (wok[u][w]) {
                    ld(pooled, o, pm[u][w]);
                    ld(dpool, o, dp[u][w]);
                }
            }
#pragma unroll
        for (int dy_ = 0; dy_ < 2; ++dy_)
#pragma unroll
            for (int dx_ = 0; dx_ < 2; ++dx_) {
                const int ih = 2 * a + dy_, iw = 2 * b + dx_;
                if (ih >= H || iw >= W) continue;
                const long pi = (((long)n * H + ih) * W + iw) * cin + ci;
                f32x4 v[QW], g[QW];
                ld(y, pi, v);
#pragma unroll
                for (int q = 0; q < QW; ++q) {
                    f32x4 z;
                    g[q] = zero;
#pragma unroll
                    for (int e = 0; e < 4; ++e) z[e] = round_to_storage<AT>(dbn_affine_relu(v[q][e], s[q][e], h[q][e]));
#pragma unroll
                    for (int u = 0; u <= dy_; ++u)
#pragma unroll
                        for (int w = 0; w <= dx_; ++w) {
                            if (!wok[u][w]) continue;
#pragma unroll
                            for (int e = 0; e < 4; ++e)
                                if (z[e] > 0.f && z[e] == pm[u][w][q][e]) g[q][e] += dp[u][w][q][e];
                        }
// ... 340 lines not shown
    }
}

__global__ void bilinear_bwd_kernel(const float* __restrict__ ddst, float* __restrict__ dsrc, long planes, int Hs, int Ws, int H, int W,
                                    float sh, float sw) {
    const long total = planes * Hs * Ws;
    for (long i = blockIdx.x * (long)blockDim.x + threadIdx.x; i < total; i += (long)gridDim.x * blockDim.x) {
        const int ws = (int)(i % Ws);
        const long t = i / Ws;
        const int hs = (int)(t % Hs);
        const long pl = t / Hs;
        const float ih = sh > 0.f ? 1.f / sh : 0.f, iw = sw > 0.f ? 1.f / sw : 0.f;
        int hlo = sh > 0.f ? (int)floorf((float)(hs - 1) * ih) - 1 : 0, hhi = sh > 0.f ? (int)ceilf((float)(hs + 1) * ih) + 1 : H - 1;
        int wlo = sw > 0.f ? (int)floorf((float)(ws - 1) * iw) - 1 : 0, whi = sw > 0.f ? (int)ceilf((float)(ws + 1) * iw) + 1 : W - 1;
        hlo = max(hlo, 0); hhi = min(hhi, H - 1);
        wlo = max(wlo, 0); whi = min(whi, W - 1);
        const float* d = ddst + pl * (long)H * W;
        float acc = 0.f;
        for (int h = hlo; h <= hhi; ++h) {
            int h0, h1;
            float lh;
            bilinear_src(h, sh, Hs, h0, h1, lh);
            const float wh = (h0 == hs ? 1.f - lh : 0.f) + (h1 == hs ? lh : 0.f);
            if (wh == 0.f) continue;
            for (int w = wlo; w <= whi; ++w) {
                int w0, w1;
                float lw;
                bilinear_src(w, sw, Ws, w0, w1, lw);
                const float ww = (w0 == ws ? 1.f - lw : 0.f) + (w1 == ws ? lw : 0.f);
                if (ww != 0.f) acc += wh * ww * d[(long)h * W + w];
            }
        }
        dsrc[i] = acc;
    }
}

__global__ void fpn_combine_weights_kernel(const float* __restrict__ w, int Co, int Cin, int g, int Cg, int f,
                                           float* __restrict__ wd) {
    const int k = f + 2;
    const long total = (long)Cg * Co * k * k;
    for (long i = blockIdx.x * (long)blockDim.x + threadIdx.x; i < total; i += (long)gridDim.x * blockDim.x) {
        const int v = (int)(i % k);
        long t = i / k;
        const int u = (int)(t % k);
        t /= k;
        const int co = (int)(t % Co);
        const int ci = (int)(t / Co);
        const float* src = w + (((long)co * Cin + g * Cg + ci) * 3) * 3;
        float acc = 0.f;
        for (int r = max(0, 2 - u); r <= min(2, f + 1 - u); ++r)
            for (int s_ = max(0, 2 - v); s_ <= min(2, f + 1 - v); ++s_) acc += src[r * 3 + s_];
        wd[i] = acc;
    }
}

__global__ void fpn_scatter_wgrad_kernel(const float* __restrict__ t0, const float* __restrict__ t1, const float* __restrict__ t2,
                                         const float* __restrict__ t3, int Co, int Cin, int Cg, float* __restrict__ dw) {
    const long total = (long)Co * Cin * 9;
    for (long i = blockIdx.x * (long)blockDim.x + threadIdx.x; i < total; i += (long)gridDim.x * blockDim.x) {
        const int s_ = (int)(i % 3);
        long t = i / 3;
        const int r = (int)(t % 3);
        t /= 3;
        const int cin = (int)(t % Cin);
        const int co = (int)(t / Cin);
        const int g = cin / Cg, ci = cin - g * Cg;
        const int f = 1 << g, k = f + 2;
        const float* tg = g == 0 ? t0 : g == 1 ? t1 : g == 2 ? t2 : t3;
        const float* base = tg + ((long)ci * Co + co) * k * k;
        float acc = 0.f;
        for (int u = 2 - r; u <= f + 1 - r; ++u)
            for (int v = 2 - s_; v <= f + 1 - s_; ++v) acc += base[u * k + v];
        dw[i] = acc;
    }
}

template <int AT>
__global__ void nchw3_to_nhwc4_kernel(const float* __restrict__ x, void* __restrict__ out, int N, long HW, int packed) {
    const long n = blockIdx.y;
    for (long p = blockIdx.x * (long)blockDim.x + threadIdx.x; p < HW; p += (long)gridDim.x * blockDim.x) {
        const long i = n * HW + p;
        const float* b = x + n * 3 * HW + p;
        const f32x4 v = {b[0], b[HW], b[2 * HW], 0.f};
        if (AT == 0 || packed) {
            dbn_st4<AT>(out, i, v);
        } else {
            const f32x4 z = {0.f, 0.f, 0.f, 0.f};
            dbn_st4<AT>(out, 4 * i, v);
            dbn_st4<AT>(out, 4 * i + 1, z);
            dbn_st4<AT>(out, 4 * i + 2, z);
            dbn_st4<AT>(out, 4 * i + 3, z);
        }
    }
}

template <int AT>
__global__ void nchw3_to_nhwc16_and_4_kernel(const float* __restrict__ x, void* __restrict__ out16, void* __restrict__ out4, int N, long HW) {
    static_assert(AT != 0, "16-bit storage");
    const long total = (long)N * HW;
    const f32x4 z = {0.f, 0.f, 0.f, 0.f};
    for (long i = blockIdx.x * (long)blockDim.x + threadIdx.x; i < total; i += (long)gridDim.x * blockDim.x) {
        const long n = i / HW, p = i - n * HW;
        const float* b = x + n * 3 * HW + p;
        const f32x4 v = {b[0], b[HW], b[2 * HW], 0.f};
        const f32x4 lo[2] = {v, z}, hi[2] = {z, z};
        dbn_stq<AT>(out16, 2 * i, lo);
        dbn_stq<AT>(out16, 2 * i + 1, hi);
        if (out4) dbn_st4<AT>(out4, i, v);
    }
}

template <int AT>
__global__ void axpy_kernel(const void* __restrict__ x, void* __restrict__ y, long total4) {
    for (long i = blockIdx.x * (long)blockDim.x + threadIdx.x; i < total4; i += (long)gridDim.x * blockDim.x)
        dbn_st4<AT>(y, i, dbn_ld4<AT>(y, i) + dbn_ld4<AT>(x, i));
}

__global__ void adam_kernel(float* __restrict__ p, const float* __restrict__ g, float* __restrict__ m, float* __restrict__ v,
                            long n, float lr_over_bc1, float b1, float b2, float eps, float inv_sqrt_bc2, float gscale) {
    const long n4 = n >> 2;
    for (long i = blockIdx.x * (long)blockDim.x + threadIdx.x; i < n4; i += (long)gridDim.x * blockDim.x) {
        f32x4 pp = reinterpret_cast<f32x4*>(p)[i];
        const f32x4 gg = reinterpret_cast<const f32x4*>(g)[i] * gscale;
        f32x4 mm = reinterpret_cast<f32x4*>(m)[i];
        f32x4 vv = reinterpret_cast<f32x4*>(v)[i];
#pragma unroll
        for (int e = 0; e < 4; ++e) {
            mm[e] = b1 * mm[e] + (1.f - b1) * gg[e];
            vv[e] = b2 * vv[e] + (1.f - b2) * gg[e] * gg[e];
            const float denom = sqrtf(vv[e]) * inv_sqrt_bc2 + eps;
            pp[e] -= lr_over_bc1 * (mm[e] / denom);
        }
        reinterpret_cast<f32x4*>(p)[i] = pp;
        reinterpret_cast<f32x4*>(m)[i] = mm;
        reinterpret_cast<f32x4*>(v)[i] = vv;
    }
    const long t = (n4 << 2) + blockIdx.x * (long)blockDim.x + threadIdx.x;
    if (t < n) {
        const float gg = g[t] * gscale;
        const float mm = b1 * m[t] + (1.f - b1) * gg;
        const float vv = b2 * v[t] + (1.f - b2) * gg * gg;
        m[t] = mm;
        v[t] = vv;
        p[t] -= lr_over_bc1 * (mm / (sqrtf(vv) * inv_sqrt_bc2 + eps));
    }
}

inline int part_blocks(int M, int C) {
    int nb = (M + 63) / 64;
    if (nb > STREAM_BLOCKS) nb = STREAM_BLOCKS;
    if (nb < 1) nb = 1;
    (void)C;
    return nb;
}
inline int bn_stream_grid(long total4, int C) {
    int g = dbn_grid(total4, 256, STREAM_BLOCKS);
    int a = C / 4, b = 256;
    while (b) { const int t = a % b; a = b; b = t; }
    const int m = (C / 4) / a;
    return (g + m - 1) / m * m;
}
inline dim3 red_grid(int nb, int C) { return dim3(nb, (C + CHUNK_C - 1) / CHUNK_C); }
inline size_t red_smem(int Cfull, int nv) {
    const int C = Cfull < CHUNK_C ? Cfull : CHUNK_C;
    const int nrl = 256 / (C / 4);
    return (size_t)(nrl > 0 ? nrl : 1) * nv * C * sizeof(float);
}

}

__global__ void clock_probe_kernel(unsigned long long* __restrict__ out, unsigned long long ref_ticks) {
    if (threadIdx.x != 0) return;
    const unsigned long long r0 = __builtin_amdgcn_s_memrealtime();
    const unsigned long long c0 = __builtin_amdgcn_s_memtime();
    unsigned long long r1 = r0;
    while (r1 - r0 < ref_ticks) {
        __builtin_amdgcn_s_sleep(64);
        r1 = __builtin_amdgcn_s_memrealtime();
    }
    const unsigned long long c1 = __builtin_amdgcn_s_memtime();
    r1 = __builtin_amdgcn_s_memrealtime();
    out[0] = c1 - c0;
    out[1] = r1 - r0;
}

extern "C" {


int dbn_reduce_ws_floats(int C) { return MAX_PART * 2 * C; }

int dbn_bn_train_stats_t(int at, const void* y, int M, int C, const float* gamma, const float* beta, float eps, float momentum,
                         float* run_mean, float* run_var, float* scale, float* shift, float* save_mean, float* save_rstd,
                         float* ws, void* stream) {
    DBN_REQUIRE(y && gamma && beta && scale && shift && save_mean && save_rstd && ws);
    DBN_REQUIRE(M > 0 && C % 4 == 0 && C >= 4 && C <= 4096 && (C <= CHUNK_C || C % CHUNK_C == 0));
    hipStream_t st = (hipStream_t)stream;
    const int nb = part_blocks(M, C);
    DBN_DISPATCH_AT(at, {
        hipLaunchKernelGGL(bn_stats_kernel<AT>, red_grid(nb, C), dim3(256), red_smem(C, 2), st, y, M, C, ws);
        hipLaunchKernelGGL(bn_finalize_kernel<AT>, dim3(dbn_ceil_div(C, 8)), dim3(256), 0, st, ws, nb, y, M, C, gamma, beta, eps,
                           momentum, run_mean, run_var, scale, shift, save_mean, save_rstd);
    });
    return dbn_status();
}
int dbn_bn_train_stats(const float* y, int M, int C, const float* gamma, const float* beta, float eps, float momentum,
                       float* run_mean, float* run_var, float* scale, float* shift, float* save_mean, float* save_rstd,
                       float* ws, void* stream) {
    return dbn_bn_train_stats_t(0, y, M, C, gamma, beta, eps, momentum, run_mean, run_var, scale, shift, save_mean, save_rstd, ws, stream);
}

int dbn_bn_eval_coef(int C, const float* gamma, const float* beta, const float* run_mean, const float* run_var, float eps,
                     float* scale, float* shift, void* stream) {
    DBN_REQUIRE(gamma && beta && run_mean && run_var && scale && shift && C > 0);
    hipLaunchKernelGGL(bn_eval_coef_kernel, dim3(dbn_ceil_div(C, 64)), dim3(64), 0, (hipStream_t)stream, C, gamma, beta,
                       run_mean, run_var, eps, scale, shift);
    return dbn_status();
}

__global__ void fold_bn_eval_kernel(const float* __restrict__ w, int O, long inner, const float* __restrict__ bias, const float* __restrict__ gamma,
                                    const float* __restrict__ beta, const float* __restrict__ mean, const float* __restrict__ var, float eps,
                                    float* __restrict__ w_out, float* __restrict__ b_out) {
    const long total = (long)O * inner;
    for (long i = blockIdx.x * (long)blockDim.x + threadIdx.x; i < total; i += (long)gridDim.x * blockDim.x) {
        const int o = (int)(i / inner);
        const float sc = gamma[o] * (1.f / sqrtf(var[o] + eps));
        w_out[i] = w[i] * sc;
        if (i - (long)o * inner == 0) b_out[o] = fmaf((bias ? bias[o] : 0.f) - mean[o], sc, beta[o]);
    }
}
int dbn_fold_bn_eval(const float* w, int O, long inner, const float* bias, const float* gamma, const float* beta, const float* run_mean,
                     const float* run_var, float eps, float* w_out, float* b_out, void* stream) {
    DBN_REQUIRE(w && gamma && beta && run_mean && run_var && w_out && b_out && O > 0 && inner > 0);
    hipLaunchKernelGGL(fold_bn_eval_kernel, dim3(dbn_grid((long)O * inner)), dim3(256), 0, (hipStream_t)stream, w, O, inner, bias, gamma, beta,
                       run_mean, run_var, eps, w_out, b_out);
    return dbn_status();
}

int dbn_bn_apply_t(int at, const void* y, const float* scale, const float* shift, const void* res, const float* res_scale,
                   const float* res_shift, void* out, long M, int C, int relu, void* stream) {
    DBN_REQUIRE(y && scale && shift && out && M > 0 && C % 4 == 0);
    DBN_REQUIRE((res_scale == nullptr) == (res_shift == nullptr));
    const long total4 = M * (C / 4);
    if (at != 0 && C % 8 == 0) {
        const long total8 = M * (C / 8);
        if (at == 1)
            hipLaunchKernelGGL((bn_apply_kernel<1, 2>), dim3(bn_stream_grid(total8, C / 2)), dim3(256), 0, (hipStream_t)stream, y, scale, shift, res,
                               res_scale, res_shift, out, total8, C, relu);
        else
            hipLaunchKernelGGL((bn_apply_kernel<2, 2>), dim3(bn_stream_grid(total8, C / 2)), dim3(256), 0, (hipStream_t)stream, y, scale, shift, res,
                               res_scale, res_shift, out, total8, C, relu);
        return dbn_status();
    }
    DBN_DISPATCH_AT(at, hipLaunchKernelGGL((bn_apply_kernel<AT, 1>), dim3(bn_stream_grid(total4, C)), dim3(256), 0, (hipStream_t)stream, y,
                                           scale, shift, res, res_scale, res_shift, out, total4, C, relu));
    return dbn_status();
}
int dbn_bn_apply(const float* y, const float* scale, const float* shift, const float* res, const float* res_scale,
                 const float* res_shift, float* out, long M, int C, int relu, void* stream) {
    return dbn_bn_apply_t(0, y, scale, shift, res, res_scale, res_shift, out, M, C, relu, stream);
}

int dbn_bn_backward_t(int at, const float* sums, int sums_parts, const void* y, const void* zmask, const float* mask_scale, const float* mask_shift,
                      const void* dout, const float* save_mean, const float* save_rstd, const float* gamma, void* dy, void* gout,
                      int gout_accumulate, float* dgamma, float* dbeta, float* dbias_conv, int M, int C, float grad_scale, float* ws,
                      void* stream) {
    DBN_REQUIRE(y && dout && save_mean && save_rstd && gamma && dy && dgamma && dbeta && ws);
    DBN_REQUIRE(!dbias_conv || 256 % (C / 4) == 0);
    DBN_REQUIRE(M > 0 && C % 4 == 0 && C >= 4 && C <= 4096 && (C <= CHUNK_C || C % CHUNK_C == 0));
    DBN_REQUIRE((mask_scale == nullptr) == (mask_shift == nullptr) && !(zmask && mask_scale));
    hipStream_t st = (hipStream_t)stream;
    const int nb = part_blocks(M, C);
    float* c1 = ws + (long)MAX_PART * 2 * C - 2 * C;
    float* c2 = c1 + C;
    const int nbu = nb < MAX_PART ? nb : MAX_PART - 1;
    const bool wide = at != 0 && C % 8 == 0 && (!dbias_conv || 256 % (C / 8) == 0);
    const long total4 = (long)M * (C / (wide ? 8 : 4));
    const int grid = bn_stream_grid(total4, wide ? C / 2 : C);
    DBN_DISPATCH_AT(at, {
        if (sums && sums_parts < 0) {
            c1 = const_cast<float*>(sums);
            c2 = c1 + C;
        } else if (sums && sums_parts >= 512) {
            hipLaunchKernelGGL(bn_bwd_finalize_wide_kernel, dim3(C), dim3(256), 0, st, sums, sums_parts, M, C, dgamma, dbeta, c1, c2,
                               grad_scale);
        } else if (sums) {
            hipLaunchKernelGGL(bn_bwd_finalize_kernel, dim3(dbn_ceil_div(C, 8)), dim3(256), 0, st, sums, sums_parts > 0 ? sums_parts : 1, M,
                               C, dgamma, dbeta, c1, c2, grad_scale);
        } else {
            hipLaunchKernelGGL(bn_bwd_reduce_kernel<AT>, red_grid(nbu, C), dim3(256), red_smem(C, 2), st, y, zmask, mask_scale,
                               mask_shift, dout, save_mean, save_rstd, M, C, ws);
            hipLaunchKernelGGL(bn_bwd_finalize_kernel, dim3(dbn_ceil_div(C, 8)), dim3(256), 0, st, ws, nbu, M, C, dgamma, dbeta, c1, c2,
                               grad_scale);
        }
#ifndef DBN_DBG_SKIP_BN_BWD_APPLY
#define DBN_DBG_SKIP_BN_BWD_APPLY 0
#endif
        if constexpr (AT != 0) {
            if (wide && !DBN_DBG_SKIP_BN_BWD_APPLY)
                hipLaunchKernelGGL((bn_bwd_apply_kernel<AT, 2>), dim3(grid), dim3(256), 0, st, y, zmask, mask_scale, mask_shift, dout, save_mean,
                                   save_rstd, gamma, c1, c2, dy, gout, gout_accumulate, total4, C, dbias_conv ? ws : nullptr);
        }
        if (!wide && !DBN_DBG_SKIP_BN_BWD_APPLY)
            hipLaunchKernelGGL((bn_bwd_apply_kernel<AT, 1>), dim3(grid), dim3(256), 0, st, y, zmask, mask_scale, mask_shift, dout, save_mean,
                               save_rstd, gamma, c1, c2, dy, gout, gout_accumulate, total4, C, dbias_conv ? ws : nullptr);
    });
    if (dbias_conv)
        hipLaunchKernelGGL(fold_partials_kernel, dim3(dbn_ceil_div(C, 8)), dim3(256), 0, st, ws, grid, C, dbias_conv, grad_scale);
    return dbn_status();
}

int dbn_bn_backward(const float* y, const float* zmask, const float* mask_scale, const float* mask_shift, const float* dout,
                    const float* save_mean, const float* save_rstd, const float* gamma, float* dy, float* gout, int gout_accumulate,
                    float* dgamma, float* dbeta, int M, int C, float grad_scale, float* ws, void* stream) {
// ... 271 lines not shown
```

db_text_minimal_amd/engine.py:

```python
import contextlib
import os

import torch

from . import _lib
from ._lib import check

DEAD_PREFIXES = ('backbone.fc.', 'backbone.smooth.')
K_STEP_DEFAULT = 50.0


def _p(t):
    return None if t is None else t.data_ptr()


def flat_layout(numels):
    offs, total = [], 0
    for n in numels:
        offs.append(total)
        total += (n + 3) // 4 * 4
    return offs, total


IGEMM_TILE_NAMES = {1: 'igemm_f32_kernel<128,128,2,2,%d,%d,%d,%s,%d,%s>', 2: 'igemm_f32_kernel<256,64,4,1,%d,%d,%d,%s,%d,%s>',
# ... 1415 lines not shown
        T = conv.k * conv.k
        vconv, ver2 = self._cols_conv(name + '.conv2', conv)
        t = self.fbuf(name + '/dw_cols', conv.cout, T * C, 1, 1)
        self.wgrad(name + '.conv2 (cols)', dy, cols, conv.cout, T * C, 1, 1, 0, t)
        check(self.L.dbn_permute_weight(t.data_ptr(), G[name + '.conv2.weight'].data_ptr(), conv.cout, C, T, 0, 1.0, self.stream),
              'permute_weight')
        dcols = self.buf(name + '/dcols', *cols.shape)
        self.conv_dgrad(name + '.conv2', dy, vconv, dcols, False, version=ver2)
        doff = self.buf(name + '/doffset', N, Ho, Wo, 64)
        slot = self._dcn_slots.setdefault(name, len(self._dcn_slots))
        if self._dcn_table is None:
            self._dcn_table = torch.zeros(64, dtype=torch.int32, device=x.device)
            self._dcn_host = torch.zeros(64, dtype=torch.int32).pin_memory()
        gather = self.dcn_gather and C <= 512 and slot < 64 and self._dcn_E.get(name, 0.0) <= self.dcn_gather_max_offset
        self.dcn_forms['gather' if gather else 'scatter'] += 1
        if gather:
            ws = self.scratch('_dcn_gather_ws', self.L.dbn_deform_col2im_gather_ws_bytes(N, Ho, Wo) // 4 + 1)
            check(self.L.dbn_deform_col2im_gather_t(self.at, dcols.data_ptr(), x.data_ptr(), off.data_ptr(), dx.data_ptr(), doff.data_ptr(),
                                                    0, ws.data_ptr(), N, H, W, C, Ho, Wo, conv.k, conv.k, conv.stride, conv.padding, 64,
                                                    self.stream), 'deform_col2im_gather')
            if slot < 64:
                self._dcn_table[slot:slot + 1].copy_(ws.view(torch.int32)[:1])
        else:
            if slot < 64:
                check(self.L.dbn_deform_offset_absmax_t(self.at, off.data_ptr(), off.numel(), self._dcn_table.data_ptr() + 4 * slot,
                                                        self.stream), 'deform_offset_absmax')
            ws = self.scratch('_dcn_col2im_ws', self.L.dbn_deform_col2im_ws_bytes(N, H, W, C, Ho, Wo, conv.k, conv.k) // 4 + 1)
            check(self.L.dbn_deform_col2im_t(self.at, dcols.data_ptr(), x.data_ptr(), off.data_ptr(), dx.data_ptr(), doff.data_ptr(), 0,
                                             ws.data_ptr(), N, H, W, C, Ho, Wo, conv.k, conv.k, conv.stride, conv.padding, 64,
                                             self.stream), 'deform_col2im')
        voc, ver = self._offset_conv(name + '.conv2_offset', oc)
        tg = self.fbuf(name + '/dw_offset', 64, C, oc.k, oc.k)
        self.wgrad(name + '.conv2_offset', doff, x, 64, C, oc.k, oc.stride, oc.padding, tg)
        nreal = oc.weight.shape[0]
        G[name + '.conv2_offset.weight'].copy_(tg[:nreal])
        tb = self.fbuf(name + '/db_offset', 64)
        self.col_sum(doff, tb)
        G[name + '.conv2_offset.bias'].copy_(tb[:nreal])
        self.conv_dgrad(name + '.conv2_offset', doff, voc, dx, True, version=ver)

    def _conv2_bn(self, name, blk, z1, train):
        if getattr(blk, 'with_dcn', False):
            return self._deform_conv_bn(name, z1, blk, name + '/y2', name + '.bn2', blk.bn2, train)
        return self.conv_bn(name + '.conv2', z1, blk.conv2, name + '/y2', name + '.bn2', blk.bn2, train)

    def _conv2_bwd(self, name, blk, dy2, z1, dz1):
        if getattr(blk, 'with_dcn', False):
            self._deform_conv_bwd(name, blk, dy2, z1, dz1)
        else:
            self.conv_wgrad(name + '.conv2', dy2, z1, blk.conv2)
            self.conv_dgrad(name + '.conv2', dy2, blk.conv2, dz1, False, consumer=(name + '.bn1', self.bufs[name + '/y1'], None))

    def _block_fwd(self, name, blk, x, train):
        if not train and self.fold_eval_bn:
            out = self._block_fwd_eval(name, blk, x)
            if out is not None:
                return out
        y1, s1, h1 = self.conv_bn(name + '.conv1', x, blk.conv1, name + '/y1', name + '.bn1', blk.bn1, train)
        if not getattr(blk, 'with_dcn', False) and self.lazy_act(y1, (blk.conv2, ), train):
            self._drop_buf(name + '/z1')
            y2, s2, h2 = self.conv_bn(name + '.conv2', y1, blk.conv2, name + '/y2', name + '.bn2', blk.bn2, train, x_act=(s1, h1))
        else:
            z1 = self.bn_apply(y1, s1, h1, name + '/z1')
            y2, s2, h2 = self._conv2_bn(name, blk, z1, train)
        if hasattr(blk, 'conv3'):
            z2 = self.bn_apply(y2, s2, h2, name + '/z2')
            ylast, s2, h2 = self.conv_bn(name + '.conv3', z2, blk.conv3, name + '/y3', name + '.bn3', blk.bn3, train)
        else:
            ylast = y2
        if blk.downsample is not None:
            yd, sd, hd = self.conv_bn(name + '.downsample.0', x, blk.downsample[0], name + '/yd', name + '.downsample.1',
                                      blk.downsample[1], train)
            out = self.bn_apply(ylast, s2, h2, name + '/out', relu=True, res=yd, rsc=sd, rsh=hd)
        else:
            out = self.bn_apply(ylast, s2, h2, name + '/out', relu=True, res=x)
        self.bufs[name + '/in'] = x
        return out

    def _block_fwd_eval(self, name, blk, x):
        convs = [(name + '.conv1', blk.conv1, blk.bn1), (name + '.conv2', blk.conv2, blk.bn2)]
        if hasattr(blk, 'conv3'):
            convs.append((name + '.conv3', blk.conv3, blk.bn3))
        if getattr(blk, 'with_dcn', False):
            return None
        cur = x
        for _, conv, _ in convs:
            if not self._fold_ok(cur, conv, False):
                return None
            N, H, W, _ = cur.shape
            cur = _Shape(N, (H + 2 * conv.padding - conv.k) // conv.stride + 1, (W + 2 * conv.padding - conv.k) // conv.stride + 1, conv.cout)
        if blk.downsample is not None and not self._fold_ok(x, blk.downsample[0], False):
            return None
        cur, res = x, x
        beside = blk.downsample is not None and self.eval_downsample_beside and self.overlap_wgrad
        if blk.downsample is not None:
            if beside:
                with self.side_stream():
                    res = self.conv_bn_act_eval(name + '.downsample.0', x, blk.downsample[0], name + '/yd', blk.downsample[1], relu=False)
            else:
                res = self.conv_bn_act_eval(name + '.downsample.0', x, blk.downsample[0], name + '/yd', blk.downsample[1], relu=False)
        for i, (cname, conv, bn) in enumerate(convs):
            last = i == len(convs) - 1
            if last and beside:
                self.join_side()
            cur = self.conv_bn_act_eval(cname, cur, conv, name + ('/out' if last else '/z%d' % (i + 1)), bn, relu=True, res=res if last else None)
        return cur

    eval_downsample_beside = os.environ.get('DBN_EVAL_DOWNSAMPLE_BESIDE', '1') == '1'

    fpn_level0_patch = int(os.environ.get('DBN_FPN_LV0_PATCH', '0'))

    def _fpn_level0_patch_ok(self, z0, Co, train=False):
        N, H, W, Cg = z0.shape
        return (self.fpn_level0_patch >= (1 if train else 2) and self.at != 0 and self.ns == 1 and Cg % 32 == 0 and H % 8 == 0 and W % 16 == 0
                and Co % 128 == 0)

    def _fpn_conv_eval(self, name, conv, zs, out_name, bn):
        N, H, W, Cg = zs[0].shape
        Co = conv.cout
        vconv, ver = self._folded(name, conv, bn)
        fname = name + '#fold'
        wds, wver = self._fpn_combined_weights(fname, vconv, Cg, version=ver)
        z = self.buf(out_name, N, H, W, Co)
        wpk = [self.pack('%s#f%d' % (fname, g), wds[g], 1, 1 << g, version=wver) for g in range(4)]
        lv0 = _VirtualConv(Cg, Co, 3, 1, 1, wds[0], vconv.bias)
        first = int(self.fpn_level0_winograd and wds[0].shape[0] == Cg and self._winograd_ok(zs[0], lv0))
        if self._fpn_level0_patch_ok(zs[0], Co):
            if self.prof:
                self._prof_igemm(N * H * W, Co, 2.0 * N * H * W * Co * Cg * 9, 'fwd %s level 0' % name, 1, (N, H, W, Cg, H, W, 3, 1, 1))
            check(self.L.dbn_igemm_act_t(self.at, self.ns, zs[0].data_ptr(), wpk[0].data_ptr(), vconv.bias.data_ptr(), None, 0, z.data_ptr(), N, H, W,
                                         Cg, H, W, Co, 3, 3, 1, 1, 1, 0, self.stream), 'igemm fpn level 0')
            if self.prof:
                self.prof.end()
            first = 1
        elif first:
            up = self._winograd_panel(fname + '#lv0', wds[0], Cg, dgrad=1, version=wver)
            if self.prof:
                self.prof.begin('winograd_f32_kernel', 2.0 * N * H * W * Co * Cg * 4, 0.0, 'fwd %s level 0' % name)
            check(self.L.dbn_winograd_conv_act_f32(zs[0].data_ptr(), up.data_ptr(), vconv.bias.data_ptr(), None, 0, z.data_ptr(), N, H, W, Cg, Co,
                                                   self.stream), 'winograd ' + name)
            if self.prof:
                self.prof.end()
        if self.prof:
            flops = sum(2.0 * N * t.shape[1] * t.shape[2] * Cg * Co * ((1 << g) + 2)**2 for g, t in enumerate(zs) if g >= first)
            bn_tile = 256 if self.L.dbn_pyramid_wide_would_run(self.at, N, H, W, Cg, Co) else 128
            waves = '1,4' if (self.at in (1, 2) and self.ns == 1) else '2,2'
            self.prof.begin('igemm_f32_kernel<128,%d,%s,3,%d,%d,false,0,true>' % (bn_tile, waves, self.ns, self.at), flops, 0.0, 'fwd %s (pyramid)' % name)
        check(self.L.dbn_pyramid_conv_act_t(first, self.at, *[t.data_ptr() for t in zs], *[w_.data_ptr() for w_ in wpk], vconv.bias.data_ptr(), 1,
                                            z.data_ptr(), N, H, W, Cg, Co, self.ns, self.stream), 'pyramid_conv_act')
        if self.prof:
            self.prof.end()
        return z

    def backward(self, dpreds):
        if self.saved_generation != self.generation:
            raise RuntimeError('backward() without a matching train-mode forward (activations were overwritten)')
        m, L, st = self.model, self.L, self.stream
        N, H, W, Hh, Wh, resample = self.saved_shape
        B = self.bufs
        self._bias_done = set()
        self._bnb_sums = {}
        self._dcn_read_back()
        self._wgrad_fifo, self._reduce_pending = [], []
        self._slab_free = [None, None]
        out = self.saved_out
        dpreds = dpreds.contiguous()
        assert dpreds.shape == (N, 3, H, W)
        if resample:
            dhead = self.fbuf('head/dout', *out.shape)
            check(L.dbn_bilinear_bwd(dpreds.data_ptr(), dhead.data_ptr(), N * 3, 2 * Hh, 2 * Wh, H, W, st), 'bilinear_bwd')
            dpreds = dhead
        head = m.segmentation_head
        b6, t6 = head.binarize[6], head.thresh[6]
        dz1b = self.buf('binarize/dz1', N, Hh, Wh, 64)
        dz1t = self.buf('thresh/dz1', N, Hh, Wh, 64)
        ws = self.scratch('_head_ws', L.dbn_head_tail_bwd_ws_floats())
        G = self.grad_views
        hb, ht = 'segmentation_head.binarize.4', 'segmentation_head.thresh.4'
        bn_sums = self.fbuf('head/bn4_sums', 4, 64)
        self._prof_hbm('head_tail_bwd_kernel + fold_head_grads_kernel + fold_partials_d_kernel', 4.0 * dz1b.element_size() * dz1b.numel() + 4.0 * (out.numel() + dpreds.numel()))
        check(L.dbn_head_tail_bwd_t(self.at, B['binarize/y1'].data_ptr(), B['thresh/y1'].data_ptr(), b6.weight.data_ptr(),
                                  t6.weight.data_ptr(), out.data_ptr(), dpreds.data_ptr(), B[hb + '/scale'].data_ptr(),
                                  B[hb + '/shift'].data_ptr(), B[ht + '/scale'].data_ptr(), B[ht + '/shift'].data_ptr(),
                                  B[hb + '/mean'].data_ptr(), B[hb + '/rstd'].data_ptr(), B[ht + '/mean'].data_ptr(),
                                  B[ht + '/rstd'].data_ptr(), bn_sums.data_ptr(), dz1b.data_ptr(), dz1t.data_ptr(),
                                  G['segmentation_head.binarize.6.weight'].data_ptr(),
                                  G['segmentation_head.binarize.6.bias'].data_ptr(),
                                  G['segmentation_head.thresh.6.weight'].data_ptr(),
                                  G['segmentation_head.thresh.6.bias'].data_ptr(), N, Hh, Wh, 3, float(head.k),
                                  self.grad_scale, ws.data_ptr(), st), 'head_tail_bwd')
        if self.prof:
            self.prof.end()
        f, f_act = B.get('fpn/z'), None
        if f is None:
            f, f_act = B['fpn/y'], (B['segmentation_body.conv.1/scale'], B['segmentation_body.conv.1/shift'])
        df = self.buf('fpn/dz', *f.shape)
        fpn = m.segmentation_body
        pre = 'segmentation_body.'
        for i, (br, dz1) in enumerate((('binarize', dz1b), ('thresh', dz1t))):
            seq = getattr(head, br)
            hp = 'segmentation_head.%s.' % br
            dy1 = self.bn_backward(hp + '4', B[br + '/y1'], 'self', dz1, br + '/dy1', sums=bn_sums[2 * i:2 * i + 2],
                                   conv_bias=hp + '3.bias' if seq[3].bias is not None else None)
            dz0 = self.buf(br + '/dz0', *B[br + '/z0'].shape)
            self.convT_bwd(hp + '3', dy1, B[br + '/z0'], seq[3], dz0, consumer=(hp + '1', B[br + '/y0'], None))
            dy0 = self.bn_backward(hp + '1', B[br + '/y0'], 'self', dz0, br + '/dy0',
                                   conv_bias=hp + '0.bias' if seq[0].bias is not None else None)
            self.conv_wgrad(hp + '0', dy0, f, seq[0], x_act=f_act)
            self.conv_dgrad(hp + '0', dy0, seq[0], df, accumulate=(i > 0),
                            consumer=(pre + 'conv.1', B['fpn/y'], None) if i > 0 else None)
        fpn = m.segmentation_body
        pre = 'segmentation_body.'
        dfy = self.bn_backward(pre + 'conv.1', B['fpn/y'], 'self', df, 'fpn/dy',
                               conv_bias=pre + 'conv.0.bias' if fpn.conv[0].bias is not None else None)
        dP = {}
        levels = ('smooth_p2', 'smooth_p3', 'smooth_p4', 'reduce_conv_c5')
        zs = [B[nm + '/z'] for nm in levels]
        if self.fpn_exact:
            self._fpn_conv_backward(pre + 'conv.0', fpn.conv[0], dfy, levels, zs, dP)
        else:
            cat = B['cat']
            self.conv_wgrad(pre + 'conv.0', dfy, cat, fpn.conv[0])
            dcat = self.buf('dcat', *cat.shape)
            self.conv_dgrad(pre + 'conv.0', dfy, fpn.conv[0], dcat, False)
            for i, nm in enumerate(levels):
                d = self.buf(nm + '/dz', *zs[i].shape)
                self.up_bwd(dcat, d, 64 * i, False)
                dP[nm] = d

        def cbr_bwd(name, mod, xin, dz, dx, dx_acc, consumer=None):
            dy = self.bn_backward(pre + name + '.bn', B[name + '/y'], 'self', dz, name + '/dy',
                                  conv_bias=pre + name + '.conv.bias' if mod.conv.bias is not None else None)
            self.conv_wgrad(pre + name + '.conv', dy, xin, mod.conv)
            self.conv_dgrad(pre + name + '.conv', dy, mod.conv, dx, dx_acc,
                            consumer=(pre + consumer + '.bn', B[consumer + '/y'], None) if consumer else None)

        lastb = {i: len(getattr(m.backbone, 'layer%d' % i)) - 1 for i in (1, 2, 3, 4)}
        feat = {i: 'backbone.layer%d.%d/out' % (i, lastb[i]) for i in (1, 2, 3, 4)}
        dC = {k: self.buf('d' + k, *B[k].shape) for k in feat.values()}
        c2, c3, c4, c5 = (B[feat[i]] for i in (1, 2, 3, 4))
        dc2, dc3, dc4, dc5 = (dC[feat[i]] for i in (1, 2, 3, 4))
        dp2pre = self.buf('dp2pre', *B['p2pre'].shape)
        cbr_bwd('smooth_p2', fpn.smooth_p2, B['p2pre'], dP['smooth_p2'], dp2pre, False, consumer='reduce_conv_c2')
        self.up_bwd(dp2pre, dP['smooth_p3'], 0, True)
        cbr_bwd('reduce_conv_c2', fpn.reduce_conv_c2, c2, dp2pre, dc2, False)
        dp3pre = self.buf('dp3pre', *B['p3pre'].shape)
        cbr_bwd('smooth_p3', fpn.smooth_p3, B['p3pre'], dP['smooth_p3'], dp3pre, False, consumer='reduce_conv_c3')
        self.up_bwd(dp3pre, dP['smooth_p4'], 0, True)
        cbr_bwd('reduce_conv_c3', fpn.reduce_conv_c3, c3, dp3pre, dc3, False)
        dp4pre = self.buf('dp4pre', *B['p4pre'].shape)
        cbr_bwd('smooth_p4', fpn.smooth_p4, B['p4pre'], dP['smooth_p4'], dp4pre, False, consumer='reduce_conv_c4')
        self.up_bwd(dp4pre, dP['reduce_conv_c5'], 0, True)
        cbr_bwd('reduce_conv_c4', fpn.reduce_conv_c4, c4, dp4pre, dc4, False)
        cbr_bwd('reduce_conv_c5', fpn.reduce_conv_c5, c5, dP['reduce_conv_c5'], dc5, False)
        self.flush_wgrad_reduces()
        if self.grad_ready_hook is not None:
            with self.side_stream():
                self._side_waits_for_reductions()
                self.grad_ready_hook('segmentation')
        bb = m.backbone
        dpool = self.buf('stem/dpool', *B['stem/pool'].shape)
        for li in (4, 3, 2, 1):
            layer = getattr(bb, 'layer%d' % li)
            for bi in range(lastb[li], -1, -1):
                name = 'backbone.layer%d.%d' % (li, bi)
                dout = self.bufs['d' + name + '/out']
                xin = B[name + '/in']
                if bi > 0:
                    dx, acc = self.buf('d' + 'backbone.layer%d.%d/out' % (li, bi - 1), *xin.shape), False
                elif li > 1:
                    dx, acc = dC[feat[li - 1]], True
                else:
                    dx, acc = dpool, False
                prev = 'backbone.layer%d.%d' % ((li, bi - 1) if bi > 0 else (li - 1, lastb[li - 1])) if (bi > 0 or li > 1) else None
                self._block_bwd(name, layer[bi], xin, dout, dx, acc, prev=prev)
            if li >= 3:
                self.flush_wgrad_reduces()
            if self.grad_ready_hook is not None and li >= 3:
                with self.side_stream():
                    self._side_waits_for_reductions()
                    self.grad_ready_hook('layer%d' % li)
        y0 = B['stem/y']
        if self.flush_before_pool:
            self._flush_wgrads()
        if self.pool_argmax and self._pool_arg_generation == self.generation:
            dy0 = self.buf('stem/dy', *y0.shape)
            ws = self.scratch('_stem_pool_bn_ws', L.dbn_maxpool_bn_backward_ws_floats(N, y0.shape[1], y0.shape[2], 64))
            es = y0.element_size()
            self._prof_hbm('maxpool_bn_stats_kernel + maxpool_bn_bwd_apply_kernel',
                           (2 * y0.numel() + 3 * dpool.numel()) * es + 2 * dpool.numel())
            check(L.dbn_maxpool_bn_backward_t(self.at, y0.data_ptr(), dpool.data_ptr(), B['stem/pool_idx'].data_ptr(), B['stem/pool_y'].data_ptr(),
                                              B['backbone.bn1/mean'].data_ptr(), B['backbone.bn1/rstd'].data_ptr(),
                                              self.views['backbone.bn1.weight'].data_ptr(), dy0.data_ptr(),
                                              self.grad_views['backbone.bn1.weight'].data_ptr(), self.grad_views['backbone.bn1.bias'].data_ptr(),
                                              N, y0.shape[1], y0.shape[2], 64, self.grad_scale, ws.data_ptr(), st), 'maxpool + bn backward')
            if self.prof:
                self.prof.end()
            self.conv_wgrad('backbone.conv1', dy0, B['x4w' if self.at != 0 else 'x4'], bb.conv1)
            self.flush_wgrad_reduces()
            self.join_side()
            self._dcn_send_back()
            self.saved_generation = -1
            self.backwards_since_clear += 1
            return
        dz = self.buf('stem/dz', *y0.shape)
        nparts = L.dbn_maxpool_bwd_parts(N, y0.shape[1], y0.shape[2], 64)
        parts = self.scratch('_stem_bn_parts', 2 * 64 * nparts)
        self._prof_hbm('bnrelu_maxpool_bwd_kernel', (2 * y0.numel() + 2 * dpool.numel()) * y0.element_size())
        check(L.dbn_bnrelu_maxpool_bwd_t(self.at, y0.data_ptr(), B['backbone.bn1/scale'].data_ptr(), B['backbone.bn1/shift'].data_ptr(),
                                         B['stem/pool'].data_ptr(), dpool.data_ptr(), dz.data_ptr(), N, y0.shape[1], y0.shape[2], 64,
                                         B['backbone.bn1/mean'].data_ptr(), B['backbone.bn1/rstd'].data_ptr(), parts.data_ptr(), st),
              'maxpool bwd')
        if self.prof:
            self.prof.end()
        dy0 = self.bn_backward('backbone.bn1', y0, None, dz, 'stem/dy', sums=parts, sums_parts=nparts)
        self.conv_wgrad('backbone.conv1', dy0, B['x4w' if self.at != 0 else 'x4'], bb.conv1)
        self.flush_wgrad_reduces()
        self.join_side()
        self._dcn_send_back()
        self.saved_generation = -1
        self.backwards_since_clear += 1

    backwards_since_clear = 0
    pool_argmax = os.environ.get('DBN_POOL_ARGMAX', '1') == '1'
    _pool_arg_generation = -1
    fpn_structured = True
    fpn_one_launch = True
    fpn_exact = False

    def _fpn_combined_weights(self, name, conv, Cg, version=None):
        w = conv.weight
        Co = w.shape[0]
        if version is None:
            self._fpn_src = (name, conv, Cg)
        stamp = (w._version if version is None else version, self.param_epoch, w.data_ptr())
        ent = self.packs.get((name, 'combined'))
        if ent is None or ent[1] != stamp:
            wds = ent[0] if ent is not None else [device_empty((Cg, Co, (1 << g) + 2, (1 << g) + 2), w.device) for g in range(4)]
            for g in range(4):
                check(self.L.dbn_fpn_combine_weights(w.data_ptr(), Co, w.shape[1], g, Cg, wds[g].data_ptr(), self.stream),
                      'fpn_combine_weights')
            self.packs[(name, 'combined')] = (wds, stamp)
        return self.packs[(name, 'combined')][0], stamp[:2]

    def _fpn_conv_forward(self, name, conv, zs, out_name, bn_name, bn, train):
        N, H, W, Cg = zs[0].shape
        Co = conv.cout
        wds, wver = self._fpn_combined_weights(name, conv, Cg)
        y = self.buf(out_name, N, H, W, Co)
        fused = train and self.fuse_bn_stats
        sc = sh = None
        if self.fpn_one_launch and Co % 128 == 0 and Cg % 16 == 0:
            wpk = [self.pack('%s#f%d' % (name, g), wds[g], 1, 1 << g, version=wver) for g in range(4)]
            lv0 = _VirtualConv(Cg, Co, 3, 1, 1, wds[0], conv.bias)
            first = int(self.fpn_level0_winograd and not self._use_planes and wds[0].shape[0] == Cg and self._winograd_ok(zs[0], lv0))
            first16 = self._fpn_level0_patch_ok(zs[0], Co, train)
# ... 139 lines not shown
```

include/dbnet_hip.h:

```cpp
#ifndef DBNET_HIP_H
#define DBNET_HIP_H
#ifdef __cplusplus
extern "C" {
#endif


int dbn_pack_weights(const float* w_oihw, int O, int I, int R, int S, int mode, int stride, float* out, void* stream);
long dbn_igemm_panel_floats(int O, int I, int R, int S, int mode, int stride);
int dbn_igemm_packed_floats(int K, int Cd);

int dbn_igemm_f32(const float* src, const float* wpk, const float* bias, float* dst, int N, int Hs, int Ws, int Cs, int Hd,
                  int Wd, int Cd, int R, int S, int stride, int pad, int mode, int accumulate, int tile_hint, void* stream);

int dbn_pack_weights_bf16s(const float* w_oihw, int O, int I, int R, int S, int mode, int stride, int ns, float* out, void* stream);
int dbn_pack_weights_batched(const void* jobs, int n, int ns, void* stream);
long dbn_igemm_bf16s_panel_floats(int O, int I, int R, int S, int mode, int stride, int ns);
int dbn_igemm_bf16s(const float* src, const float* wpk, const float* bias, float* dst, int N, int Hs, int Ws, int Cs, int Hd,
                    int Wd, int Cd, int R, int S, int stride, int pad, int mode, int accumulate, int tile_hint, int ns,
                    void* stream);
int dbn_wgrad_bf16s(const float* sm, const float* big, float* slab, float* grad_oihw, int N, int Ho, int Wo, int O, int H, int W,
                    int Cb, int I, int R, int S, int stride, int pad, float scale, int ns, void* stream);

int dbn_igemm_bn_rows(int at, int ns, int N, int Hs, int Ws, int Cs, int Hd, int Wd, int Cd, int R, int S, int stride, int pad, int mode,
                      int tile_hint);
// ... 211 lines not shown
long dbn_detect_poly_verts_cap(int N, int H, int W);
int dbn_detect_poly(const float* pred, int N, int channels, int H, int W, float thresh, int max_candidates, void* ws, void* poly_ws,
                    int* labels, void* table, short* verts, void* stream);
int dbn_detect_poly_host(const void* recs, const int* counts, const int* nv, const int* voff, const short* verts, int N, int max_candidates,
                         int H, int W, const double* params, const int* dest_hw, int* poly_n, int* poly_off, int* poly_xy, int poly_cap,
                         int* poly_total, double* scores, double* info, int* approx_xy);

long dbn_det_eval_ws_bytes(int n_polys);
int dbn_det_eval_overlaps(const double* verts, const int* poff, int n_polys, const long long* img, int N, long n_pairs, int cull, void* ws,
                          double* inter, double* area, int* nonsimple, void* stream);
int dbn_det_eval_match_host(int protocol, int N, const int* sizes, const double* inter, const double* gt_area, const double* det_area,
                            const unsigned char* gt_ignore, const double* gt_cd, const double* det_cd, const double* params, double* stats,
                            unsigned char* det_dc, int* rows, int* n_rows);


#define DBN_AT_F32 0
#define DBN_AT_BF16 1
#define DBN_AT_F16 2
#define DBN_AT_SPLIT3 3
int dbn_split3(const float* src, void* planes, long n, void* stream);

long dbn_igemm_panel_floats_t(int kind, int O, int I, int R, int S, int mode, int stride, int cs);
int dbn_pack_weights_t(int kind, const float* w_oihw, int O, int I, int R, int S, int mode, int stride, int cs, float* out, void* stream);

int dbn_igemm_t(int at, int ns, const void* src, const float* wpk, const float* bias, void* dst, int N, int Hs, int Ws, int Cs, int Hd,
                int Wd, int Cd, int R, int S, int stride, int pad, int mode, int accumulate, int tile_hint, int ksplit, float* slab,
                void* stream);
int dbn_conv_bn_t(int at, const void* src, const float* wpk, const float* bias, void* dst, int N, int Hs, int Ws, int Cs, int Hd, int Wd,
                  int Cd, int R, int S, int stride, int pad, int mode, int accumulate, int tile_hint, int ns,
                  const float* gamma, const float* beta, float eps, float momentum, float* run_mean, float* run_var,
                  float* scale, float* shift, float* save_mean, float* save_rstd, float* ws, void* stream);
int dbn_pyramid_conv_t(int at, const void* s0, const void* s1, const void* s2, const void* s3, const float* w0, const float* w1,
                       const float* w2, const float* w3, const float* bias, void* dst, int N, int H, int W, int Cs, int Cd,
                       int tile_hint, int ns, const float* gamma, const float* beta, float eps, float momentum, float* run_mean,
                       float* run_var, float* scale, float* shift, float* save_mean, float* save_rstd, float* ws, void* stream);
int dbn_pyramid_conv_from_t(int first_level, int at, const void* s0, const void* s1, const void* s2, const void* s3, const float* w0,
                            const float* w1, const float* w2, const float* w3, const float* bias, void* dst, int N, int H, int W, int Cs,
                            int Cd, int tile_hint, int ns, const float* gamma, const float* beta, float eps, float momentum,
                            float* run_mean, float* run_var, float* scale, float* shift, float* save_mean, float* save_rstd, float* ws,
                            void* stream);
int dbn_wgrad_t(int at, int ns, const void* sm, const void* big, float* slab, float* grad_oihw, int N, int Ho, int Wo, int O, int H, int W,
                int Cb, int I, int R, int S, int stride, int pad, float scale, void* stream);

int dbn_set_wgrad_variant(int variant);
int dbn_set_convt_kernel(int on);
int dbn_wgrad_kernel_config(int at, int ns, int O, int J, int Cb);
int dbn_wgrad_kernel_config_hw(int at, int ns, int O, int Cb, int R, int S, int stride, int pad, int Ho, int Wo, int H, int W);
int dbn_set_patch_conv(int on);
int dbn_set_wres16(int on);
int dbn_set_pyramid_wide(int on);
int dbn_pyramid_wide_would_run(int at, int N, int H, int W, int Cs, int Cd);
int dbn_wres16_would_run(int at, int mode, int N, int H, int W, int Cs, int Cd, int bnb, int y2);

int dbn_mfma_sustained(int kind, const void* operands, float* out, int iters, void* stream);
long dbn_mfma_sustained_flops(int kind, int iters);
int dbn_set_stagger(int permille);
int dbn_set_phase_priority(int on);
int dbn_set_trace(void* buf, long max_blocks);
int dbn_igemm_kernel_config(int at, int ns, int kmode, int N, int Hs, int Ws, int Cs, int Hd, int Wd, int Cd, int R, int S, int stride,
                            int pad, int tile_hint, int ksplit);
typedef struct dbn_wgrad_reduce_job {
    const float* slab;
    float* grad;
    int splitk, O, J, Jp, BM, BN, Cb, I, RS, G, natural, blocks;
    float scale;
    int smem_bytes;
} dbn_wgrad_reduce_job;
int dbn_wgrad_reduce_describe(int at, int ns, const void* sm, const void* big, float* slab, float* grad_oihw, int N, int Ho, int Wo, int O,
                              int H, int W, int Cb, int I, int R, int S, int stride, int pad, float scale, void* job);
int dbn_wgrad_reduce_many(const void* jobs, const int* first, int n_jobs, int total_blocks, int max_smem, void* stream);
int dbn_wgrad_tile_config(int O, int J);
int dbn_wgrad_phase_t(int phase, int at, int ns, const void* sm, const void* big, float* slab, float* grad_oihw, int N, int Ho, int Wo,
                      int O, int H, int W, int Cb, int I, int R, int S, int stride, int pad, float scale, void* stream);

int dbn_deform_im2col_t(int at, const void* x, const void* offset, void* cols, int N, int H, int W, int C, int Ho, int Wo, int R, int S,
                        int stride, int pad, int off_stride, void* stream);
int dbn_deform_col2im_t(int at, const void* dcols, const void* x, const void* offset, void* dx, void* doffset, int accumulate, void* ws,
                        int N, int H, int W, int C, int Ho, int Wo, int R, int S, int stride, int pad, int off_stride, void* stream);
long dbn_deform_col2im_gather_ws_bytes(int N, int Ho, int Wo);
int dbn_deform_col2im_gather_t(int at, const void* dcols, const void* x, const void* offset, void* dx, void* doffset, int accumulate,
                               void* ws, int N, int H, int W, int C, int Ho, int Wo, int R, int S, int stride, int pad, int off_stride,
                               void* stream);
int dbn_deform_offset_absmax_t(int at, const void* offset, long n, unsigned* out_bits, void* stream);
int dbn_cast_f32(int at, const float* src, void* dst, long n, void* stream);

int dbn_bn_train_stats_t(int at, const void* y, int M, int C, const float* gamma, const float* beta, float eps, float momentum,
                         float* run_mean, float* run_var, float* scale, float* shift, float* save_mean, float* save_rstd,
                         float* ws, void* stream);
int dbn_bn_apply_t(int at, const void* y, const float* scale, const float* shift, const void* res, const float* res_scale,
                   const float* res_shift, void* out, long M, int C, int relu, void* stream);
int dbn_bn_backward_t(int at, const float* sums, int sums_parts, const void* y, const void* zmask, const float* mask_scale,
                      const float* mask_shift, const void* dout, const float* save_mean, const float* save_rstd, const float* gamma,
                      void* dy, void* gout, int gout_accumulate, float* dgamma, float* dbeta, float* dbias_conv, int M, int C,
                      float grad_scale, float* ws, void* stream);
int dbn_col_sum_t(int at, const void* x, int M, int C, float* out, float scale, float* ws, void* stream);
int dbn_bnrelu_maxpool_fwd_t(int at, const void* y, const float* scale, const float* shift, void* out, int N, int H, int W, int C,
                             void* stream);
int dbn_maxpool_bwd_parts(int N, int H, int W, int C);
int dbn_bnrelu_maxpool_bwd_t(int at, const void* y, const float* scale, const float* shift, const void* pooled, const void* dpool,
                             void* dz, int N, int H, int W, int C, const float* bn_mean, const float* bn_rstd, float* bn_part,
                             void* stream);
int dbn_bnrelu_maxpool_fwd_arg_t(int at, const void* y, const float* scale, const float* shift, void* out, void* idx, void* ypool, int N, int H,
                                 int W, int C, void* stream);
long dbn_maxpool_bn_backward_ws_floats(int N, int H, int W, int C);
int dbn_maxpool_bn_backward_t(int at, const void* y, const void* dpool, const void* idx, const void* ypool, const float* save_mean,
                              const float* save_rstd, const float* gamma, void* dy, float* dgamma, float* dbeta, int N, int H, int W, int C,
                              float grad_scale, float* ws, void* stream);
int dbn_nearest_up_fwd_t(int at, const void* src, const void* addend, void* dst, int N, int Hs, int Ws, int C, int H, int W, int Cdst,
                         int coff, void* stream);
int dbn_nearest_up_bwd_t(int at, const void* dbig, void* dsrc, int N, int Hs, int Ws, int C, int H, int W, int Cbig, int coff,
                         int accumulate, void* stream);
int dbn_nchw3_to_nhwc4_t(int at, const float* x, void* out, int N, int H, int W, void* stream);
int dbn_stem16_padded_h(int H);
int dbn_stem16_padded_w(int W);
int dbn_stem16_rows(void);
long dbn_stem16_panel_bytes(void);
int dbn_stem16_eligible(int at, int N, int H, int W);
int dbn_stem16_pack(int kind, const float* w_oihw, void* out, void* stream);
int dbn_nchw3_to_padded4_t(int at, const float* x, void* xp, void* x4, int N, int H, int W, void* stream);
int dbn_stem16_conv_bn_t(int at, const void* xp, const void* wpk, void* y, int N, int H, int W, const float* gamma, const float* beta, float eps,
                         float momentum, float* run_mean, float* run_var, float* scale, float* shift, float* save_mean, float* save_rstd,
                         float* ws, void* stream);
int dbn_stem16_pool_eligible(int at, int N, int H, int W);
int dbn_stem16_conv_bn_relu_pool_t(int at, const void* xp, const void* wpk, const float* scale, const float* shift, void* out, int N, int H, int W,
                                   void* stream);
int dbn_convt16_rows(void);
long dbn_convt16_panel_bytes(void);
int dbn_convt16_eligible(int at, int N, int H, int W, int Cin, int Cout);
int dbn_convt16_pack(int kind, const float* w_iohw, void* out, void* stream);
int dbn_convt16_bn_t(int at, const void* x, const void* wpk, const float* bias, void* y, int N, int H, int W, const float* gamma, const float* beta,
                     float eps, float momentum, float* run_mean, float* run_var, float* scale, float* shift, float* save_mean, float* save_rstd,
                     float* ws, void* stream);
int dbn_pw16_eligible(int at, int N, int H, int W, int Cin, int Cout);
long dbn_pw16_panel_bytes(void);
int dbn_pw16_pack(int kind, const float* w_oihw, int Cout, void* out, void* stream);
int dbn_pw16_act_t(int at, const void* x, const void* wpk, const float* bias, int relu, void* y, int N, int H, int W, int Cout, void* stream);
int dbn_head16_eligible(int at, int N, int Hq, int Wq);
int dbn_head16_tail_eval_t(int at, const void* x_b, const void* x_t, const void* panel_b, const void* panel_t, const float* bias1_b,
                           const float* bias1_t, const float* scale_b, const float* shift_b, const float* scale_t, const float* shift_t,
                           const float* w2_b, const float* w2_t, const float* bias2_b, const float* bias2_t, float* out, int N, int Hq, int Wq,
                           void* stream);

int dbn_nchw3_to_nhwc16_and_4_t(int at, const float* x, void* out16, void* out4, int N, int H, int W, void* stream);
int dbn_nchw3_to_nhwc4_packed_t(int at, const float* x, void* out, int N, int H, int W, void* stream);
int dbn_head_tail_fwd_t(int at, const void* xb, const void* xt, const float* wb, const float* wt, const float* bias_b,
                        const float* bias_t, const float* bn_scale_b, const float* bn_shift_b, const float* bn_scale_t,
                        const float* bn_shift_t, float* out, int N, int Hq, int Wq, int channels, float kstep, void* stream);
int dbn_set_head_tail_wide(int mode);
int dbn_head_tail_bwd_t(int at, const void* xb, const void* xt, const float* wb, const float* wt, const float* preds,
                        const float* dpreds, const float* bn_scale_b, const float* bn_shift_b, const float* bn_scale_t,
                        const float* bn_shift_t, const float* bn_mean_b, const float* bn_rstd_b, const float* bn_mean_t,
                        const float* bn_rstd_t, float* bn_sums, void* dxb, void* dxt, float* dw_b, float* dbias_b, float* dw_t,
                        float* dbias_t, int N, int Hq, int Wq, int channels, float kstep, float grad_scale, float* ws, void* stream);

int dbn_jpeg_info(const unsigned char* data, long len, long long* out);
int dbn_jpeg_info_ex(const unsigned char* data, long len, int flags, long long* out);
long dbn_jpeg_coef_elems_ex(const unsigned char* blob, const long long* offs, int N, int flags, long long* per_image);
int dbn_jpeg_entropy_batch_ex(const unsigned char* blob, const long long* offs, int N, short* coef, long coef_elems, long long* desc,
                              unsigned short* qtabs, int* status, int* orientation, int threads, int flags);
int dbn_jpeg_pixels_ex(const short* coef, long coef_elems, const long long* desc, const unsigned short* qtabs, int N, const int* tab_idct,
                       int n_idct, const int* tab_rgb, int n_rgb, const int* orientation, const int* tab_tile, int n_tile,
                       unsigned char* planes, unsigned char* out, long out_bytes, void* stream);
long dbn_jpeg_coef_elems(const unsigned char* blob, const long long* offs, int N, long long* per_image);
int dbn_jpeg_entropy_batch(const unsigned char* blob, const long long* offs, int N, short* coef, long coef_elems, long long* desc,
                           unsigned short* qtabs, int* status, int threads);
int dbn_jpeg_pixels(const short* coef, long coef_elems, const long long* desc, const unsigned short* qtabs, int N, const int* tab_idct,
                    int n_idct, const int* tab_rgb, int n_rgb, unsigned char* planes, unsigned char* out, long out_bytes, void* stream);

int dbn_jpeg_forward(const unsigned char* pixels, long in_bytes, const long long* desc, const unsigned short* qtabs, int N,
                     const int* tab_planes, int n_planes, const int* tab_fdct, int n_fdct, unsigned char* planes, short* coef, long coef_elems,
                     void* stream);
long dbn_jpeg_encode_bound(const long long* desc, int N, int restart_interval, long long* per_image);
int dbn_jpeg_encode_batch(const short* coef, long coef_elems, const long long* desc, const unsigned short* qtabs, int N, int restart_interval,
                          unsigned char* out, long out_bytes, const long long* offs, long long* lens, int* status, int threads);
int dbn_jpeg_optimal_table(const long long* freq, unsigned char* bits, unsigned char* vals, int* nvals);
int dbn_jpeg_encode_batch_opt(const short* coef, long coef_elems, const long long* desc, const unsigned short* qtabs, int N, int restart_interval,
                              unsigned char* out, long out_bytes, const long long* offs, long long* lens, int* status, int threads, int optimize);

int dbn_jpeg_huff_plan(const long long* desc, const unsigned short* qtabs, int N, long coef_elems, int restart_interval, long long* blk_base,
                       long long* int_base, int* status, long long* sizes);
int dbn_jpeg_huff_hist(const short* coef, long coef_elems, const long long* desc, int N, const long long* blk_base, long total_blocks,
                       int restart_interval, unsigned* hist, unsigned long long* errkey, void* stream);
int dbn_jpeg_huff_annex_k(unsigned short* specs, unsigned* codes);
int dbn_jpeg_huff_tables(const unsigned* hist, const long long* desc, int N, int* status, unsigned short* specs, unsigned* codes, int threads);
int dbn_jpeg_huff_code(const short* coef, long coef_elems, const long long* desc, int N, const long long* blk_base, const long long* int_base,
                       long total_blocks, long total_intervals, int restart_interval, const unsigned* codes, int per_image, void* ws, long ws_bytes,
                       unsigned char* out, long out_bytes, unsigned long long* res, void* stream);
int dbn_jpeg_huff_headers(const long long* desc, const unsigned short* qtabs, int N, int restart_interval, const unsigned short* specs, int per_image,
                          const int* status, unsigned char* out, long long* lens);

int dbn_jpeg_stream_plan(const unsigned char* blob, const long long* offs, int N, long long* desc, unsigned short* qtabs, int* status,
                         unsigned char* hspec, long long* info, long long* seg, long seg_cap, long long* sub_base, int* wgtab, long wg_cap,
                         long long* counts);
long dbn_jpeg_dhuff_ws_bytes(long nsub);
int dbn_jpeg_dhuff(const unsigned char* blob, long blob_len, const long long* desc, const unsigned char* hspec, const long long* info,
                   const long long* seg, const long long* sub_base, const int* wgtab, int N, long nseg, long nsub, int nwg, int rounds, short* coef,
                   long coef_elems, void* ws, long ws_bytes, unsigned long long* res, void* stream);

#ifdef __cplusplus
}
#endif
#endif
```

Measured before the change: 736.8.

## Fuse head tail backward with BN backward, recomputing gradient instead of storing dz1

Adds a fused head-tail plus BatchNorm backward path. A sums-only pass computes the BN statistics without writing the dz1 intermediate. An apply pass then recomputes the upstream gradient from preds/dpreds and the 1x1 head weights, and writes dy1 directly while also folding the conv bias gradient. This removes one full-size write and read of dz1 per branch, at the cost of redoing the small per-pixel gradient math and reading the prediction maps twice. The fused path is gated on a flag and the activation type, with the old path kept as a fallback.

```diff
diff --git a/db_text_minimal_amd/_lib.py b/db_text_minimal_amd/_lib.py
--- a/db_text_minimal_amd/_lib.py
+++ b/db_text_minimal_amd/_lib.py
@@ -222,6 +222,8 @@
     'dbn_stem16_conv_bn_t': 'ipppiii' + 'pp' + 'ff' + 'ppppppp' + 'p',
     'dbn_head_tail_fwd_t': 'i' + SIGNATURES['dbn_head_tail_fwd'],
     'dbn_head_tail_bwd_t': 'i' + SIGNATURES['dbn_head_tail_bwd'],
+    'dbn_head_tail_bn_bwd_ws_floats': '',
+    'dbn_head_tail_bn_bwd_t': 'ii' + 'p' * 28 + 'iiii' + 'ff' + 'pp',
 })
 LONG_RETURN = {'dbn_jpeg_coef_elems', 'dbn_jpeg_coef_elems_ex', 'dbn_jpeg_dhuff_ws_bytes', 'dbn_jpeg_encode_bound', 'dbn_greedy_decode_ws_bytes', 'dbn_det_eval_ws_bytes', 'dbn_detect_ws_bytes', 'dbn_detect_poly_ws_bytes', 'dbn_detect_poly_verts_cap', 'dbn_mfma_sustained_flops', 'dbn_conv_bn_final_group_doubles', 'dbn_maxpool_bn_backward_ws_floats', 'dbn_pw16_panel_bytes', 'dbn_stem16_panel_bytes', 'dbn_convt16_panel_bytes', 'dbn_winograd_panel_floats', 'dbn_winograd_wgrad_slab_floats', 'dbn_winograd_ws_floats', 'dbn_igemm_splitk_slab_floats', 'dbn_deform_col2im_ws_bytes', 'dbn_deform_col2im_gather_ws_bytes', 'dbn_igemm_bn_final_counters', 'dbn_igemm_bn_final_group_floats', 'dbn_igemm_panel_floats_t', 'dbn_wgrad_slab_floats_hw', 'dbn_wgrad_slab_floats', 'dbn_igemm_panel_floats', 'dbn_igemm_bf16s_panel_floats', 'dbn_db_loss_ohem_ws_bytes', 'dbn_conv_bn_ws_floats', 'dbn_pyramid_conv_ws_floats'}
 _KIND = {'p': _P, 'i': _I, 'l': _L, 'f': _F}
diff --git a/db_text_minimal_amd/csrc/bn_bwd_apply.h b/db_text_minimal_amd/csrc/bn_bwd_apply.h
--- /dev/null
+++ b/db_text_minimal_amd/csrc/bn_bwd_apply.h
@@ -0,0 +1,152 @@
+#pragma once
+#include "common.h"
+
+namespace {
+
+constexpr int STREAM_BLOCKS = 768;
+constexpr int UNROLL = 4;
+
+inline int bn_stream_grid(long total4, int C) {
+    int g = dbn_grid(total4, 256, STREAM_BLOCKS);
+    int a = C / 4, b = 256;
+    while (b) { const int t = a % b; a = b; b = t; }
+    const int m = (C / 4) / a;
+    return (g + m - 1) / m * m;
+}
+
+template <int AT>
+__device__ __forceinline__ float round_to_storage(float v) {
+    if constexpr (AT == 1) return (float)(__bf16)v;
+    else if constexpr (AT == 2) return (float)(_Float16)v;
+    else return v;
+}
+
+template <int AT, int QW>
+struct BnGradStored {
+    const void* __restrict__ dout;
+    struct Raw { f32x4 g[QW]; };
+    __device__ __forceinline__ void fetch(long i, Raw& r) const {
+        if constexpr (QW == 1) r.g[0] = dbn_ld4<AT>(dout, i);
+        else dbn_ldq<AT>(dout, i, r.g);
+    }
+    __device__ __forceinline__ void grad(const Raw& r, f32x4 (&g)[QW]) const {
+#pragma unroll
+        for (int q = 0; q < QW; ++q) g[q] = r.g[q];
+    }
+};
+
+template <int AT, int QW, class SRC>
+__device__ __forceinline__ void bn_bwd_apply_body(const void* __restrict__ y, const void* __restrict__ zmask, const float* __restrict__ msc,
+                                                  const float* __restrict__ msh, SRC& src, const float* __restrict__ mean,
+                                                  const float* __restrict__ rstd, const float* __restrict__ gamma,
+                                                  const float* __restrict__ c1, const float* __restrict__ c2, void* __restrict__ dy,
+                                                  void* __restrict__ gout, int gout_acc, long total, int C, float* __restrict__ bias_part) {
+    static_assert(QW == 1 || (QW == 2 && AT != 0), "two quads per access: 16-bit storage");
+    const int cin = C / (4 * QW);
+    const long i0 = blockIdx.x * (long)blockDim.x + threadIdx.x;
+    const long stride = (long)gridDim.x * blockDim.x;
+    const int c = (int)(i0 % cin) * 4 * QW;
+    const f32x4 zero = {0.f, 0.f, 0.f, 0.f};
+    f32x4 s_[QW], h_[QW], mu[QW], rs[QW], k1[QW], k2[QW], gr[QW], bsum[QW];
+#pragma unroll
+    for (int q = 0; q < QW; ++q) {
+        s_[q] = h_[q] = zero;
+        if (msc) {
+            s_[q] = *reinterpret_cast<const f32x4*>(msc + c + 4 * q);
+            h_[q] = *reinterpret_cast<const f32x4*>(msh + c + 4 * q);
+        }
+        mu[q] = *reinterpret_cast<const f32x4*>(mean + c + 4 * q);
+        rs[q] = *reinterpret_cast<const f32x4*>(rstd + c + 4 * q);
+        k1[q] = *reinterpret_cast<const f32x4*>(c1 + c + 4 * q);
+        k2[q] = *reinterpret_cast<const f32x4*>(c2 + c + 4 * q);
+        gr[q] = *reinterpret_cast<const f32x4*>(gamma + c + 4 * q) * rs[q];
+        bsum[q] = zero;
+    }
+    const bool acc = gout && gout_acc;
+    auto ld = [&](const void* ptr, long i, f32x4 (&v)[QW]) {
+        if constexpr (QW == 1) v[0] = dbn_ld4<AT>(ptr, i);
+        else dbn_ldq<AT>(ptr, i, v);
+    };
+    auto st = [&](void* ptr, long i, const f32x4 (&v)[QW]) {
+        if constexpr (QW == 1) dbn_st4<AT>(ptr, i, v[0]);
+        else dbn_stq<AT>(ptr, i, v);
+    };
+    auto one = [&](long i, const typename SRC::Raw& raw, const f32x4 (&v)[QW], const f32x4 (&z)[QW], const f32x4 (&old)[QW]) {
+        f32x4 g[QW], d[QW], go[QW];
+        src.grad(raw, g);
+#pragma unroll
+        for (int q = 0; q < QW; ++q) {
+            if (zmask) {
+#pragma unroll
+                for (int e = 0; e < 4; ++e) g[q][e] = z[q][e] > 0.f ? g[q][e] : 0.f;
+            } else if (msc) {
+#pragma unroll
+                for (int e = 0; e < 4; ++e) g[q][e] = dbn_affine(v[q][e], s_[q][e], h_[q][e]) > 0.f ? g[q][e] : 0.f;
+            }
+            const f32x4 xh = (v[q] - mu[q]) * rs[q];
+            d[q] = gr[q] * (g[q] - k1[q] - xh * k2[q]);
+#pragma unroll
+            for (int e = 0; e < 4; ++e) {
+                float t = d[q][e];
+                asm("" : "+v"(t));
+                d[q][e] = round_to_storage<AT>(t);
+            }
+            bsum[q] += d[q];
+            go[q] = acc ? g[q] + old[q] : g[q];
+        }
+        st(dy, i, d);
+        if (gout) st(gout, i, go);
+    };
+    auto zeros = [&](f32x4 (&v)[QW]) {
+#pragma unroll
+        for (int q = 0; q < QW; ++q) v[q] = zero;
+    };
+    long i = i0;
+    for (; i + (UNROLL - 1) * stride < total; i += UNROLL * stride) {
+        typename SRC::Raw g[UNROLL];
+        f32x4 v[UNROLL][QW], z[UNROLL][QW], o[UNROLL][QW];
+#pragma unroll
+        for (int u = 0; u < UNROLL; ++u) {
+            src.fetch(i + u * stride, g[u]);
+            ld(y, i + u * stride, v[u]);
+        }
+#pragma unroll
+        for (int u = 0; u < UNROLL; ++u) {
+            if (zmask) ld(zmask, i + u * stride, z[u]);
+            else zeros(z[u]);
+            if (acc) ld(gout, i + u * stride, o[u]);
+            else zeros(o[u]);
+        }
+#pragma unroll
+        for (int u = 0; u < UNROLL; ++u) one(i + u * stride, g[u], v[u], z[u], o[u]);
+    }
+    for (; i < total; i += stride) {
+        typename SRC::Raw g;
+        f32x4 v[QW], z[QW], o[QW];
+        src.fetch(i, g);
+        ld(y, i, v);
+        if (zmask) ld(zmask, i, z);
+        else zeros(z);
+        if (acc) ld(gout, i, o);
+        else zeros(o);
+        one(i, g, v, z, o);
+    }
+    if (bias_part) {
+        __shared__ f32x4 red[QW][256];
+#pragma unroll
+        for (int q = 0; q < QW; ++q) red[q][threadIdx.x] = bsum[q];
+        __syncthreads();
+        if ((int)threadIdx.x < cin) {
+            const int cq = (int)((blockIdx.x * (long)blockDim.x + threadIdx.x) % cin) * 4 * QW;
+#pragma unroll
+            for (int q = 0; q < QW; ++q) {
+                f32x4 t = zero;
+                for (int k = threadIdx.x; k < 256; k += cin) t += red[q][k];
+#pragma unroll
+                for (int e = 0; e < 4; ++e) bias_part[(long)(cq + 4 * q + e) * gridDim.x + blockIdx.x] = t[e];
+            }
+        }
+    }
+}
+
+}
diff --git a/db_text_minimal_amd/csrc/head_loss.hip b/db_text_minimal_amd/csrc/head_loss.hip
--- a/db_text_minimal_amd/csrc/head_loss.hip
+++ b/db_text_minimal_amd/csrc/head_loss.hip
@@ -1,4 +1,5 @@
 #include "common.h"
+#include "bn_bwd_apply.h"
 
 namespace {
 
@@ -160,7 +161,10 @@
 #else
 #define DBN_HT_OCC
 #endif
-template <int AT>
+#ifndef DBN_HT_SUMS_UNROLL
+#define DBN_HT_SUMS_UNROLL 2
+#endif
+template <int AT, bool STORE = true, int U = 1>
 __global__ __launch_bounds__(256) DBN_HT_OCC void head_tail_bwd_kernel(const void* __restrict__ xb, const void* __restrict__ xt, const float* __restrict__ wb,
                                      const float* __restrict__ wt, const float* __restrict__ preds,
                                      const float* __restrict__ dpreds, const float* __restrict__ sc_b,
@@ -218,18 +222,31 @@
         if (hq >= Hq) { hq -= Hq; ++n; }
         n += g_n;
     };
-    for (long px = px0; px < npx; px += gstride, advance()) {
+    struct Raw { float P, T, dP, dT, B, dB; f32x4 vb, vt; };
+    auto fetch = [&](long px, Raw& r) {
+        const int ab = q & 3;
+        const long o = (long)(2 * hq + (ab >> 1)) * W + 2 * wq + (ab & 1);
+        const float* pb = preds + n * CH * HW + o;
+        const float* db = dpreds + n * CH * HW + o;
+        r.P = pb[0], r.T = pb[HW];
+        r.dP = db[0], r.dT = db[HW];
+        r.B = r.dB = 0.f;
+        if (CH == 3) {
+            r.B = pb[2 * HW];
+            r.dB = db[2 * HW];
+        }
+        r.vb = dbn_ld4<AT>(xb, px * 16 + q);
+        r.vt = dbn_ld4<AT>(xt, px * 16 + q);
+        advance();
+    };
+    auto work = [&](long px, const Raw& r) {
         float dlb = 0.f, dlt = 0.f;
         {
-            const int ab = q & 3;
-            const long o = (long)(2 * hq + (ab >> 1)) * W + 2 * wq + (ab & 1);
-            const float* pb = preds + n * CH * HW + o;
-            const float* db = dpreds + n * CH * HW + o;
-            const float P = pb[0], T = pb[HW];
-            float dP = db[0], dT = db[HW];
+            const float P = r.P, T = r.T;
+            float dP = r.dP, dT = r.dT;
             if (CH == 3) {
-                const float B = pb[2 * HW];
-                const float gB = db[2 * HW] * kstep * B * (1.f - B);
+                const float B = r.B;
+                const float gB = r.dB * kstep * B * (1.f - B);
                 dP += gB;
                 dT -= gB;
             }
@@ -238,8 +255,8 @@
         }
         const f32x4 lb = {quad_bcast<0>(dlb), quad_bcast<1>(dlb), quad_bcast<2>(dlb), quad_bcast<3>(dlb)};
         const f32x4 lt = {quad_bcast<0>(dlt), quad_bcast<1>(dlt), quad_bcast<2>(dlt), quad_bcast<3>(dlt)};
-        f32x4 vb = dbn_ld4<AT>(xb, px * 16 + q);
-        f32x4 vt = dbn_ld4<AT>(xt, px * 16 + q);
+        f32x4 vb = r.vb;
+        f32x4 vt = r.vt;
         const f32x4 yb = vb, yt = vt;
         if (bn) {
 #pragma unroll
@@ -256,14 +273,21 @@
             awb[e] += vb[e] * lb;
             awt[e] += vt[e] * lt;
         }
-        dbn_st4<AT>(dxb, px * 16 + q, gb);
-        dbn_st4<AT>(dxt, px * 16 + q, gt);
+        if constexpr (STORE) {
+            dbn_st4<AT>(dxb, px * 16 + q, gb);
+            dbn_st4<AT>(dxt, px * 16 + q, gt);
+        }
         if (bnsum) {
             if constexpr (AT != 0) {
 #pragma unroll
                 for (int e = 0; e < 4; ++e) {
-                    gb[e] = AT == 1 ? (float)(__bf16)gb[e] : (float)(_Float16)gb[e];
-                    gt[e] = AT == 1 ? (float)(__bf16)gt[e] : (float)(_Float16)gt[e];
+                    float fb = gb[e], ft = gt[e];
+                    if constexpr (!STORE) {
+                        asm("" : "+v"(fb));
+                        asm("" : "+v"(ft));
+                    }
+                    gb[e] = AT == 1 ? (float)(__bf16)fb : (float)(_Float16)fb;
+                    gt[e] = AT == 1 ? (float)(__bf16)ft : (float)(_Float16)ft;
                 }
             }
 #pragma unroll
@@ -279,6 +303,21 @@
             abb += lb[0] + lb[1] + lb[2] + lb[3];
             abt += lt[0] + lt[1] + lt[2] + lt[3];
         }
+    };
+    long px = px0;
+    if constexpr (U > 1) {
+        for (; px + (U - 1) * gstride < npx; px += U * gstride) {
+            Raw r[U];
+#pragma unroll
+            for (int u = 0; u < U; ++u) fetch(px + u * gstride, r[u]);
+#pragma unroll
+            for (int u = 0; u < U; ++u) work(px + u * gstride, r[u]);
+        }
+    }
+    for (; px < npx; px += gstride) {
+        Raw r;
+        fetch(px, r);
+        work(px, r);
     }
 #if DBN_HT_CHECK
     {
@@ -356,6 +395,114 @@
     const int j = i < 257 ? i : i - 257;
     float* dst = i < 257 ? (j < 256 ? dw_b + j : dbias_b) : (j < 256 ? dw_t + j : dbias_t);
     *dst = (float)(s * scale);
+}
+
+template <int AT, int QW>
+struct HeadGradRecomputed {
+    struct Raw { float p, d, B, dB; };
+    const float* __restrict__ preds;
+    const float* __restrict__ dpreds;
+    f32x4 w[4 * QW];
+    long n, HW, plane;
+    int hq, wq, Hq, Wq, W, CH, br, ab;
+    long g_n;
+    int g_h, g_w;
+    float kstep;
+    __device__ __forceinline__ HeadGradRecomputed(const float* __restrict__ preds_, const float* __restrict__ dpreds_, const float* __restrict__ wgt,
+                                                  int br_, int Hq_, int Wq_, int CH_, float kstep_)
+        : preds(preds_), dpreds(dpreds_), Hq(Hq_), Wq(Wq_), CH(CH_), br(br_), kstep(kstep_) {
+        constexpr int cin = 16 / QW;
+        const long i0 = blockIdx.x * (long)blockDim.x + threadIdx.x;
+        const long gstride = (long)gridDim.x * blockDim.x / cin;
+        const int c = (int)(i0 % cin) * 4 * QW;
+#pragma unroll
+        for (int e = 0; e < 4 * QW; ++e) w[e] = *reinterpret_cast<const f32x4*>(wgt + (c + e) * 4);
+        W = 2 * Wq;
+        HW = (long)(2 * Hq) * W;
+        plane = br * HW;
+        ab = threadIdx.x & 3;
+        const long px0 = i0 / cin, HWq = (long)Hq * Wq;
+        n = px0 / HWq;
+        hq = (int)((px0 - n * HWq) / Wq);
+        wq = (int)((px0 - n * HWq) - (long)hq * Wq);
+        g_n = gstride / HWq;
+        g_h = (int)((gstride - g_n * HWq) / Wq);
+        g_w = (int)((gstride - g_n * HWq) - (long)g_h * Wq);
+    }
+    __device__ __forceinline__ void fetch(long, Raw& r) {
+        const long o = (long)(2 * hq + (ab >> 1)) * W + 2 * wq + (ab & 1);
+        const float* pb = preds + n * CH * HW + o;
+        const float* db = dpreds + n * CH * HW + o;
+        r.p = pb[plane];
+        r.d = db[plane];
+        r.B = r.dB = 0.f;
+        if (CH == 3) {
+            r.B = pb[2 * HW];
+            r.dB = db[2 * HW];
+        }
+        wq += g_w;
+        if (wq >= Wq) { wq -= Wq; ++hq; }
+        hq += g_h;
+        if (hq >= Hq) { hq -= Hq; ++n; }
+        n += g_n;
+    }
+    __device__ __forceinline__ void grad(const Raw& r, f32x4 (&g)[QW]) const {
+        float d = r.d;
+        if (CH == 3) {
+            const float gB = r.dB * kstep * r.B * (1.f - r.B);
+            if (br) d -= gB;
+            else d += gB;
+        }
+        const float dl = d * r.p * (1.f - r.p);
+        const f32x4 l = {quad_bcast<0>(dl), quad_bcast<1>(dl), quad_bcast<2>(dl), quad_bcast<3>(dl)};
+#pragma unroll
+        for (int q = 0; q < QW; ++q)
+#pragma unroll
+            for (int e = 0; e < 4; ++e) {
+                float t = w[4 * q + e][0] * l[0] + w[4 * q + e][1] * l[1] + w[4 * q + e][2] * l[2] + w[4 * q + e][3] * l[3];
+                if constexpr (AT != 0) asm("" : "+v"(t));
+                g[q][e] = round_to_storage<AT>(t);
+            }
+    }
+};
+
+struct HeadBnBranch {
+    const void* y;
+    const float *scale, *shift, *mean, *rstd, *gamma, *c1, *c2;
+    const float* w;
+    void* dy;
+    float* bias_part;
+};
+
+template <int AT, int QW>
+__global__ __launch_bounds__(256) void head_bn_bwd_apply_kernel(HeadBnBranch b0, HeadBnBranch b1, const float* __restrict__ preds,
+                                                                const float* __restrict__ dpreds, int Hq, int Wq, int CH, float kstep,
+                                                                long total) {
+    const int br = blockIdx.y;
+    const HeadBnBranch b = br ? b1 : b0;
+    HeadGradRecomputed<AT, QW> src(preds, dpreds, b.w, br, Hq, Wq, CH, kstep);
+    bn_bwd_apply_body<AT, QW>(b.y, nullptr, b.scale, b.shift, src, b.mean, b.rstd, b.gamma, b.c1, b.c2, b.dy, nullptr, 0, total, 64, b.bias_part);
+}
+
+__global__ void head_bn_bwd_finalize_kernel(const float* __restrict__ sums, int M, float* __restrict__ dgamma_b, float* __restrict__ dbeta_b,
+                                            float* __restrict__ dgamma_t, float* __restrict__ dbeta_t, float* __restrict__ cc, float gscale) {
+    const int i = threadIdx.x;
+    if (i >= 128) return;
+    const int br = i >> 6, c = i & 63;
+    const double s1 = (double)sums[br * 128 + c], s2 = (double)sums[br * 128 + 64 + c];
+    (br ? dbeta_t : dbeta_b)[c] = (float)(s1 * gscale);
+    (br ? dgamma_t : dgamma_b)[c] = (float)(s2 * gscale);
+    cc[br * 128 + c] = (float)(s1 / M);
+    cc[br * 128 + 64 + c] = (float)(s2 / M);
+}
+
+__global__ void fold_head_bias_kernel(const float* __restrict__ part_b, const float* __restrict__ part_t, int nb, float* __restrict__ out_b,
+                                      float* __restrict__ out_t, float scale) {
+    const int i = blockIdx.x * 8 + (threadIdx.x >> 5);
+    const int l32 = threadIdx.x & 31;
+    if (i >= 128) return;
+    const double s = dbn_team32_fold(i < 64 ? part_b : part_t, nb, i & 63, l32);
+    if (l32 == 0) (i < 64 ? out_b : out_t)[i & 63] = (float)(s * scale);
 }
 
 enum { S_POS = 0, S_NEG, S_BCE, S_L1, S_A, S_BGM, S_BM, S_NONBIN , NSUM };
@@ -862,6 +1009,56 @@
                                grad_scale, ws, stream);
 }
 
+static const long HEAD_BN_WS_SUMS = 2048L * (2 * 257 + 4 * 64), HEAD_BN_WS_CC = HEAD_BN_WS_SUMS + 256, HEAD_BN_WS_BIAS = HEAD_BN_WS_CC + 256;
+int dbn_head_tail_bn_bwd_ws_floats() { return (int)(HEAD_BN_WS_BIAS + 2L * 64 * STREAM_BLOCKS); }
+
+int dbn_head_tail_bn_bwd_t(int at, int phases, const void* yb, const void* yt, const float* wb, const float* wt, const float* preds, const float* dpreds,
+                           const float* bn_scale_b, const float* bn_shift_b, const float* bn_scale_t, const float* bn_shift_t,
+                           const float* bn_mean_b, const float* bn_rstd_b, const float* bn_mean_t, const float* bn_rstd_t,
+                           const float* bn_gamma_b, const float* bn_gamma_t, void* dyb, void* dyt, float* dgamma_b, float* dbeta_b,
+                           float* dgamma_t, float* dbeta_t, float* dbias_conv_b, float* dbias_conv_t, float* dw_b, float* dbias_b, float* dw_t,
+                           float* dbias_t, int N, int Hq, int Wq, int channels, float kstep, float grad_scale, float* ws, void* stream) {
+    DBN_REQUIRE(yb && yt && wb && wt && preds && dpreds && dyb && dyt && dw_b && dbias_b && dw_t && dbias_t && ws);
+    DBN_REQUIRE(bn_scale_b && bn_shift_b && bn_scale_t && bn_shift_t && bn_mean_b && bn_rstd_b && bn_mean_t && bn_rstd_t && bn_gamma_b && bn_gamma_t);
+    DBN_REQUIRE(dgamma_b && dbeta_b && dgamma_t && dbeta_t && (dbias_conv_b == nullptr) == (dbias_conv_t == nullptr));
+    DBN_REQUIRE((channels == 2 || channels == 3) && N > 0 && Hq > 0 && Wq > 0 && (long)N * Hq * Wq <= 0x7fffffffL);
+    DBN_REQUIRE(phases >= 1 && phases <= 3 && at >= 0 && at <= 2);
+    hipStream_t st = (hipStream_t)stream;
+    const long npx = (long)N * Hq * Wq;
+    const int nb = dbn_grid(npx * 16, 256, 2047);
+    float* sums = ws + HEAD_BN_WS_SUMS;
+    float* cc = ws + HEAD_BN_WS_CC;
+    if (phases & 1) {
+        DBN_DISPATCH_AT(at, hipLaunchKernelGGL((head_tail_bwd_kernel<AT, false, DBN_HT_SUMS_UNROLL>), dim3(nb), dim3(256), 0, st, yb, yt, wb, wt, preds, dpreds, bn_scale_b,
+                                               bn_shift_b, bn_scale_t, bn_shift_t, bn_mean_b, bn_rstd_b, bn_mean_t, bn_rstd_t, (void*)nullptr,
+                                               (void*)nullptr, ws, N, Hq, Wq, channels, kstep));
+        hipLaunchKernelGGL(fold_head_grads_kernel, dim3(dbn_ceil_div(2 * 257, 8)), dim3(256), 0, st, ws, nb, dw_b, dbias_b, dw_t, dbias_t,
+                           grad_scale);
+        hipLaunchKernelGGL(fold_partials_d_kernel, dim3(dbn_ceil_div(256, 8)), dim3(256), 0, st, ws + (long)514 * nb, nb, 256, sums, 1.0f);
+        hipLaunchKernelGGL(head_bn_bwd_finalize_kernel, dim3(1), dim3(128), 0, st, sums, (int)npx, dgamma_b, dbeta_b, dgamma_t, dbeta_t, cc, grad_scale);
+    }
+    if (!(phases & 2)) return dbn_status();
+    const int qw = at == 0 ? 1 : 2;
+    const long total = npx * (16 / qw);
+    const int grid = bn_stream_grid(total, 64 / qw);
+    DBN_REQUIRE(grid <= STREAM_BLOCKS);
+    const bool bias = dbias_conv_b != nullptr;
+    float* bias_part = ws + HEAD_BN_WS_BIAS;
+    const HeadBnBranch b0 = {yb, bn_scale_b, bn_shift_b, bn_mean_b, bn_rstd_b, bn_gamma_b, cc, cc + 64, wb, dyb, bias ? bias_part : nullptr};
+    const HeadBnBranch b1 = {yt, bn_scale_t, bn_shift_t, bn_mean_t, bn_rstd_t, bn_gamma_t, cc + 128, cc + 192, wt, dyt,
+                             bias ? bias_part + 64L * grid : nullptr};
+    if (at == 0)
+        hipLaunchKernelGGL((head_bn_bwd_apply_kernel<0, 1>), dim3(grid, 2), dim3(256), 0, st, b0, b1, preds, dpreds, Hq, Wq, channels, kstep, total);
+    else if (at == 1)
+        hipLaunchKernelGGL((head_bn_bwd_apply_kernel<1, 2>), dim3(grid, 2), dim3(256), 0, st, b0, b1, preds, dpreds, Hq, Wq, channels, kstep, total);
+    else
+        hipLaunchKernelGGL((head_bn_bwd_apply_kernel<2, 2>), dim3(grid, 2), dim3(256), 0, st, b0, b1, preds, dpreds, Hq, Wq, channels, kstep, total);
+    if (bias)
+        hipLaunchKernelGGL(fold_head_bias_kernel, dim3(dbn_ceil_div(128, 8)), dim3(256), 0, st, bias_part, bias_part + 64L * grid, grid, dbias_conv_b,
+                           dbias_conv_t, grad_scale);
+    return dbn_status();
+}
+
 static const long DB_LOSS_PART_BYTES = 1024L * NSUM * 8;
 int dbn_db_loss_ws_bytes() { return (int)DB_LOSS_PART_BYTES + 64; }
 
diff --git a/db_text_minimal_amd/csrc/pointwise.hip b/db_text_minimal_amd/csrc/pointwise.hip
--- a/db_text_minimal_amd/csrc/pointwise.hip
+++ b/db_text_minimal_amd/csrc/pointwise.hip
@@ -1,10 +1,9 @@
 #include "common.h"
+#include "bn_bwd_apply.h"
 
 namespace {
 
 constexpr int MAX_PART = 1024;
-constexpr int STREAM_BLOCKS = 768;
-constexpr int UNROLL = 4;
 
 constexpr int CHUNK_C = 1024;
 
@@ -248,13 +247,6 @@
     c2[c] = (float)(s2 / M);
 }
 
-template <int AT>
-__device__ __forceinline__ float round_to_storage(float v) {
-    if constexpr (AT == 1) return (float)(__bf16)v;
-    else if constexpr (AT == 2) return (float)(_Float16)v;
-    else return v;
-}
-
 template <int AT, int QW>
 __global__ __launch_bounds__(256) void bn_bwd_apply_kernel(const void* __restrict__ y, const void* __restrict__ zmask,
                                                            const float* __restrict__ msc, const float* __restrict__ msh,
@@ -263,109 +255,8 @@
                                                            const float* __restrict__ c1, const float* __restrict__ c2,
                                                            void* __restrict__ dy, void* __restrict__ gout, int gout_acc,
                                                            long total, int C, float* __restrict__ bias_part) {
-    static_assert(QW == 1 || (QW == 2 && AT != 0), "two quads per access: 16-bit storage");
-    const int cin = C / (4 * QW);
-    const long i0 = blockIdx.x * (long)blockDim.x + threadIdx.x;
-    const long stride = (long)gridDim.x * blockDim.x;
-    const int c = (int)(i0 % cin) * 4 * QW;
-    const f32x4 zero = {0.f, 0.f, 0.f, 0.f};
-    f32x4 s_[QW], h_[QW], mu[QW], rs[QW], k1[QW], k2[QW], gr[QW], bsum[QW];
-#pragma unroll
-    for (int q = 0; q < QW; ++q) {
-        s_[q] = h_[q] = zero;
-        if (msc) {
-            s_[q] = *reinterpret_cast<const f32x4*>(msc + c + 4 * q);
-            h_[q] = *reinterpret_cast<const f32x4*>(msh + c + 4 * q);
-        }
-        mu[q] = *reinterpret_cast<const f32x4*>(mean + c + 4 * q);
-        rs[q] = *reinterpret_cast<const f32x4*>(rstd + c + 4 * q);
-        k1[q] = *reinterpret_cast<const f32x4*>(c1 + c + 4 * q);
-        k2[q] = *reinterpret_cast<const f32x4*>(c2 + c + 4 * q);
-        gr[q] = *reinterpret_cast<const f32x4*>(gamma + c + 4 * q) * rs[q];
-        bsum[q] = zero;
-    }
-    const bool acc = gout && gout_acc;
-    auto ld = [&](const void* ptr, long i, f32x4 (&v)[QW]) {
-        if constexpr (QW == 1) v[0] = dbn_ld4<AT>(ptr, i);
-        else dbn_ldq<AT>(ptr, i, v);
-    };
-    auto st = [&](void* ptr, long i, const f32x4 (&v)[QW]) {
-        if constexpr (QW == 1) dbn_st4<AT>(ptr, i, v[0]);
-        else dbn_stq<AT>(ptr, i, v);
-    };
-    auto one = [&](long i, f32x4 (&g)[QW], const f32x4 (&v)[QW], const f32x4 (&z)[QW], const f32x4 (&old)[QW]) {
-        f32x4 d[QW], go[QW];
-#pragma unroll
-        for (int q = 0; q < QW; ++q) {
-            if (zmask) {
-#pragma unroll
-                for (int e = 0; e < 4; ++e) g[q][e] = z[q][e] > 0.f ? g[q][e] : 0.f;
-            } else if (msc) {
-#pragma unroll
-                for (int e = 0; e < 4; ++e) g[q][e] = dbn_affine(v[q][e], s_[q][e], h_[q][e]) > 0.f ? g[q][e] : 0.f;
-            }
-            const f32x4 xh = (v[q] - mu[q]) * rs[q];
-            d[q] = gr[q] * (g[q] - k1[q] - xh * k2[q]);
-#pragma unroll
-            for (int e = 0; e < 4; ++e) {
-                float t = d[q][e];
-                asm("" : "+v"(t));
-                d[q][e] = round_to_storage<AT>(t);
-            }
-            bsum[q] += d[q];
-            go[q] = acc ? g[q] + old[q] : g[q];
-        }
-        st(dy, i, d);
-        if (gout) st(gout, i, go);
-    };
-    auto zeros = [&](f32x4 (&v)[QW]) {
-#pragma unroll
-        for (int q = 0; q < QW; ++q) v[q] = zero;
-    };
-    long i = i0;
-    for (; i + (UNROLL - 1) * stride < total; i += UNROLL * stride) {
-        f32x4 g[UNROLL][QW], v[UNROLL][QW], z[UNROLL][QW], o[UNROLL][QW];
-#pragma unroll
-        for (int u = 0; u < UNROLL; ++u) {
-            ld(dout, i + u * stride, g[u]);
-            ld(y, i + u * stride, v[u]);
-        }
-#pragma unroll
-        for (int u = 0; u < UNROLL; ++u) {
-            if (zmask) ld(zmask, i + u * stride, z[u]);
-            else zeros(z[u]);
-            if (acc) ld(gout, i + u * stride, o[u]);
-            else zeros(o[u]);
-        }
-#pragma unroll
-        for (int u = 0; u < UNROLL; ++u) one(i + u * stride, g[u], v[u], z[u], o[u]);
-    }
-    for (; i < total; i += stride) {
-        f32x4 g[QW], v[QW], z[QW], o[QW];
-        ld(dout, i, g);
-        ld(y, i, v);
-        if (zmask) ld(zmask, i, z);
-        else zeros(z);
-        if (acc) ld(gout, i, o);
-        else zeros(o);
-        one(i, g, v, z, o);
-    }
-    if (bias_part) {
-        __shared__ f32x4 red[QW][256];
-#pragma unroll
-        for (int q = 0; q < QW; ++q) red[q][threadIdx.x] = bsum[q];
-        __syncthreads();
-        if ((int)threadIdx.x < cin) {
-            const int cq = (int)((blockIdx.x * (long)blockDim.x + threadIdx.x) % cin) * 4 * QW;
-#pragma unroll
-            for (int q = 0; q < QW; ++q) {
-                f32x4 t = zero;
-                for (int k = threadIdx.x; k < 256; k += cin) t += red[q][k];
-#pragma unroll
-                for (int e = 0; e < 4; ++e) bias_part[(long)(cq + 4 * q + e) * gridDim.x + blockIdx.x] = t[e];
-            }
-        }
-    }
+    BnGradStored<AT, QW> src{dout};
+    bn_bwd_apply_body<AT, QW>(y, zmask, msc, msh, src, mean, rstd, gamma, c1, c2, dy, gout, gout_acc, total, C, bias_part);
 }
 
 template <int AT>
@@ -1012,13 +903,6 @@
     if (nb < 1) nb = 1;
     (void)C;
     return nb;
-}
-inline int bn_stream_grid(long total4, int C) {
-    int g = dbn_grid(total4, 256, STREAM_BLOCKS);
-    int a = C / 4, b = 256;
-    while (b) { const int t = a % b; a = b; b = t; }
-    const int m = (C / 4) / a;
-    return (g + m - 1) / m * m;
 }
 inline dim3 red_grid(int nb, int C) { return dim3(nb, (C + CHUNK_C - 1) / CHUNK_C); }
 inline size_t red_smem(int Cfull, int nv) {
diff --git a/db_text_minimal_amd/engine.py b/db_text_minimal_amd/engine.py
--- a/db_text_minimal_amd/engine.py
+++ b/db_text_minimal_amd/engine.py
@@ -1591,6 +1591,63 @@
             self.prof.end()
         return z
 
+    head_bwd_fused = os.environ.get('DBN_HEAD_BWD_FUSED', '1') == '1'
+    head_bwd_fused_ats = (0, 1, 2)
+
+    def _head_tail_args(self, out, dpreds):
+        B, head = self.bufs, self.model.segmentation_head
+        hb, ht = 'segmentation_head.binarize.4', 'segmentation_head.thresh.4'
+        return (B['binarize/y1'].data_ptr(), B['thresh/y1'].data_ptr(), head.binarize[6].weight.data_ptr(), head.thresh[6].weight.data_ptr(),
+                out.data_ptr(), dpreds.data_ptr(), B[hb + '/scale'].data_ptr(), B[hb + '/shift'].data_ptr(), B[ht + '/scale'].data_ptr(),
+                B[ht + '/shift'].data_ptr(), B[hb + '/mean'].data_ptr(), B[hb + '/rstd'].data_ptr(), B[ht + '/mean'].data_ptr(),
+                B[ht + '/rstd'].data_ptr())
+
+    def _head_tail_grads(self):
+        G = self.grad_views
+        return tuple(G['segmentation_head.%s.6.%s' % (br, k)].data_ptr() for br in ('binarize', 'thresh') for k in ('weight', 'bias'))
+
+    def _head_tail_bwd(self, out, dpreds, N, Hh, Wh):
+        L, head = self.L, self.model.segmentation_head
+        dz1b = self.buf('binarize/dz1', N, Hh, Wh, 64)
+        dz1t = self.buf('thresh/dz1', N, Hh, Wh, 64)
+        ws = self.scratch('_head_ws', L.dbn_head_tail_bwd_ws_floats())
+        bn_sums = self.fbuf('head/bn4_sums', 4, 64)
+        self._prof_hbm('head_tail_bwd_kernel + fold_head_grads_kernel + fold_partials_d_kernel', 4.0 * dz1b.element_size() * dz1b.numel() + 4.0 * (out.numel() + dpreds.numel()))
+        check(L.dbn_head_tail_bwd_t(self.at, *self._head_tail_args(out, dpreds), bn_sums.data_ptr(), dz1b.data_ptr(), dz1t.data_ptr(),
+                                    *self._head_tail_grads(), N, Hh, Wh, 3, float(head.k), self.grad_scale, ws.data_ptr(), self.stream),
+              'head_tail_bwd')
+        if self.prof:
+            self.prof.end()
+        return dz1b, dz1t, bn_sums
+
+    def _head_tail_bn_bwd(self, out, dpreds, N, Hh, Wh):
+        L, B, G, head = self.L, self.bufs, self.grad_views, self.model.segmentation_head
+        y1b, y1t = B['binarize/y1'], B['thresh/y1']
+        dyb, dyt = self.buf('binarize/dy1', *y1b.shape), self.buf('thresh/dy1', *y1t.shape)
+        ws = self.scratch('_head_bn_ws', L.dbn_head_tail_bn_bwd_ws_floats())
+        hp = ['segmentation_head.%s.' % br for br in ('binarize', 'thresh')]
+        dbias = [None, None]
+        biased = [getattr(head, br)[3].bias is not None for br in ('binarize', 'thresh')]
+        if all(biased) and self.bias_grad_in_bn:
+            for i in (0, 1):
+                dbias[i] = G[hp[i] + '3.bias'].data_ptr()
+                self._bias_done.add(hp[i] + '3.bias')
+        T, maps = y1b.numel() * y1b.element_size(), 4.0 * (out.numel() + dpreds.numel())
+        args = (*self._head_tail_args(out, dpreds), self.views[hp[0] + '4.weight'].data_ptr(), self.views[hp[1] + '4.weight'].data_ptr(),
+                dyb.data_ptr(), dyt.data_ptr(), G[hp[0] + '4.weight'].data_ptr(), G[hp[0] + '4.bias'].data_ptr(),
+                G[hp[1] + '4.weight'].data_ptr(), G[hp[1] + '4.bias'].data_ptr(), dbias[0], dbias[1], *self._head_tail_grads(), N, Hh, Wh, 3,
+                float(head.k), self.grad_scale, ws.data_ptr(), self.stream)
+        self._prof_hbm('head_tail_bwd_kernel + fold_head_grads_kernel + fold_partials_d_kernel', 2.0 * T + maps, 'sums only')
+        check(L.dbn_head_tail_bn_bwd_t(self.at, 1, *args), 'head_tail_bn_bwd (sums)')
+        if self.prof:
+            self.prof.end()
+        self._prof_hbm('bn_bwd_reduce_kernel + bn_bwd_finalize_kernel + bn_bwd_apply_kernel', 4.0 * T + maps * 8.0 / 6.0,
+                       'segmentation_head.{binarize,thresh}.4 [recomputed gradient]')
+        check(L.dbn_head_tail_bn_bwd_t(self.at, 2, *args), 'head_tail_bn_bwd (apply)')
+        if self.prof:
+            self.prof.end()
+        return dyb, dyt
+
     def backward(self, dpreds):
         if self.saved_generation != self.generation:
             raise RuntimeError('backward() without a matching train-mode forward (activations were overwritten)')
@@ -1610,37 +1667,28 @@
             check(L.dbn_bilinear_bwd(dpreds.data_ptr(), dhead.data_ptr(), N * 3, 2 * Hh, 2 * Wh, H, W, st), 'bilinear_bwd')
             dpreds = dhead
         head = m.segmentation_head
-        b6, t6 = head.binarize[6], head.thresh[6]
-        dz1b = self.buf('binarize/dz1', N, Hh, Wh, 64)
-        dz1t = self.buf('thresh/dz1', N, Hh, Wh, 64)
-        ws = self.scratch('_head_ws', L.dbn_head_tail_bwd_ws_floats())
-        G = self.grad_views
         hb, ht = 'segmentation_head.binarize.4', 'segmentation_head.thresh.4'
-        bn_sums = self.fbuf('head/bn4_sums', 4, 64)
-        self._prof_hbm('head_tail_bwd_kernel + fold_head_grads_kernel + fold_partials_d_kernel', 4.0 * dz1b.element_size() * dz1b.numel() + 4.0 * (out.numel() + dpreds.numel()))
-        check(L.dbn_head_tail_bwd_t(self.at, B['binarize/y1'].data_ptr(), B['thresh/y1'].data_ptr(), b6.weight.data_ptr(),
-                                  t6.weight.data_ptr(), out.data_ptr(), dpreds.data_ptr(), B[hb + '/scale'].data_ptr(),
-                                  B[hb + '/shift'].data_ptr(), B[ht + '/scale'].data_ptr(), B[ht + '/shift'].data_ptr(),
-                                  B[hb + '/mean'].data_ptr(), B[hb + '/rstd'].data_ptr(), B[ht + '/mean'].data_ptr(),
-                                  B[ht + '/rstd'].data_ptr(), bn_sums.data_ptr(), dz1b.data_ptr(), dz1t.data_ptr(),
-                                  G['segmentation_head.binarize.6.weight'].data_ptr(),
-                                  G['segmentation_head.binarize.6.bias'].data_ptr(),
-                                  G['segmentation_head.thresh.6.weight'].data_ptr(),
-                                  G['segmentation_head.thresh.6.bias'].data_ptr(), N, Hh, Wh, 3, float(head.k),
-                                  self.grad_scale, ws.data_ptr(), st), 'head_tail_bwd')
-        if self.prof:
-            self.prof.end()
+        fused = self.head_bwd_fused and self.at in self.head_bwd_fused_ats and all(
+            h + k in B for h in (hb, ht) for k in ('/scale', '/shift', '/mean', '/rstd'))
+        head_dy1 = self._head_tail_bn_bwd(out, dpreds, N, Hh, Wh) if fused else None
+        if not fused:
+            head_dy1 = self._head_tail_bwd(out, dpreds, N, Hh, Wh)
         f, f_act = B.get('fpn/z'), None
         if f is None:
             f, f_act = B['fpn/y'], (B['segmentation_body.conv.1/scale'], B['segmentation_body.conv.1/shift'])
         df = self.buf('fpn/dz', *f.shape)
         fpn = m.segmentation_body
         pre = 'segmentation_body.'
-        for i, (br, dz1) in enumerate((('binarize', dz1b), ('thresh', dz1t))):
+        for i, br in enumerate(('binarize', 'thresh')):
             seq = getattr(head, br)
             hp = 'segmentation_head.%s.' % br
-            dy1 = self.bn_backward(hp + '4', B[br + '/y1'], 'self', dz1, br + '/dy1', sums=bn_sums[2 * i:2 * i + 2],
-                                   conv_bias=hp + '3.bias' if seq[3].bias is not None else None)
+            if fused:
+                self._flush_wgrads()
+                dy1 = head_dy1[i]
+            else:
+                dz1, bn_sums = head_dy1[i], head_dy1[2]
+                dy1 = self.bn_backward(hp + '4', B[br + '/y1'], 'self', dz1, br + '/dy1', sums=bn_sums[2 * i:2 * i + 2],
+                                       conv_bias=hp + '3.bias' if seq[3].bias is not None else None)
             dz0 = self.buf(br + '/dz0', *B[br + '/z0'].shape)
             self.convT_bwd(hp + '3', dy1, B[br + '/z0'], seq[3], dz0, consumer=(hp + '1', B[br + '/y0'], None))
             dy0 = self.bn_backward(hp + '1', B[br + '/y0'], 'self', dz0, br + '/dy0',
diff --git a/include/dbnet_hip.h b/include/dbnet_hip.h
--- a/include/dbnet_hip.h
+++ b/include/dbnet_hip.h
@@ -387,6 +387,13 @@
                         const float* bn_shift_t, const float* bn_mean_b, const float* bn_rstd_b, const float* bn_mean_t,
                         const float* bn_rstd_t, float* bn_sums, void* dxb, void* dxt, float* dw_b, float* dbias_b, float* dw_t,
                         float* dbias_t, int N, int Hq, int Wq, int channels, float kstep, float grad_scale, float* ws, void* stream);
+int dbn_head_tail_bn_bwd_ws_floats(void);
+int dbn_head_tail_bn_bwd_t(int at, int phases, const void* yb, const void* yt, const float* wb, const float* wt, const float* preds, const float* dpreds,
+                           const float* bn_scale_b, const float* bn_shift_b, const float* bn_scale_t, const float* bn_shift_t,
+                           const float* bn_mean_b, const float* bn_rstd_b, const float* bn_mean_t, const float* bn_rstd_t,
+                           const float* bn_gamma_b, const float* bn_gamma_t, void* dyb, void* dyt, float* dgamma_b, float* dbeta_b,
+                           float* dgamma_t, float* dbeta_t, float* dbias_conv_b, float* dbias_conv_t, float* dw_b, float* dbias_b, float* dw_t,
+                           float* dbias_t, int N, int Hq, int Wq, int channels, float kstep, float grad_scale, float* ws, void* stream);
 
 int dbn_jpeg_info(const unsigned char* data, long len, long long* out);
 int dbn_jpeg_info_ex(const unsigned char* data, long len, int flags, long long* out);
```

Result: faster. 747.3, median of 6 (+1.4%).
